# dexmal/dexbotic

Hardware: AMD Instinct MI355X
Metric: episodes/sec DB-CogACT fine-tune (higher is better)
Workload: dtype bf16; 1 GPU; DB-CogACT fine-tune step (CLIP-L/14@224 x1 view, Qwen2.5-7B-class 28L decoder, DiT-B head, AdamW), 16 episodes/GPU, 32-token instruction, S=287; global_batch=16, seq_len=287, parallelism=dp1, optimizer=AdamW serial, grad_accum=1, activations=resident

## Files before the change

### dexbotic_amd/csrc/gemm.hip

```cpp
#include "common.h"
#include "gemm_common.h"

#include <algorithm>

namespace {


template <typename T> struct EltTraits;
template <> struct EltTraits<float> { static constexpr int EPC = 4; };
template <> struct EltTraits<bf16_t> { static constexpr int EPC = 8; };

__device__ __forceinline__ int lds_off(int row, int chunk) { return row * ROWB + ((chunk ^ (row & 7)) << 4); }

template <typename T, int NR>
__device__ __forceinline__ void load_kc(uint4 (&r)[4], const T* __restrict__ base, int64_t ld, int64_t row0,
                                        int64_t rows, int64_t k0, int64_t K, int vec, int tid) {
  constexpr int EPC = EltTraits<T>::EPC;
  const int c = tid & 7;
  const int64_t k = k0 + (int64_t)c * EPC;
#pragma unroll
  for (int i = 0; i < NR / 32; ++i) {
    const int64_t row = row0 + (tid >> 3) + 32 * i;
    uint4 v = make_uint4(0, 0, 0, 0);
    if (row < rows && k < K) {
      const T* p = base + row * ld + k;
      if (vec && k + EPC <= K) {
        v = *reinterpret_cast<const uint4*>(p);
      } else {
        alignas(16) T tmp[EPC];
#pragma unroll
        for (int e = 0; e < EPC; ++e) tmp[e] = (k + e < K) ? p[e] : (T)0;
        v = *reinterpret_cast<const uint4*>(tmp);
      }
    }
    r[i] = v;
  }
}
template <int NR>
__device__ __forceinline__ void store_kc(const uint4 (&r)[4], char* tile, int tid) {
  const int c = tid & 7;
#pragma unroll
  for (int i = 0; i < NR / 32; ++i) {
    const int row = (tid >> 3) + 32 * i;
    *reinterpret_cast<uint4*>(tile + lds_off(row, c)) = r[i];
  }
}

template <typename T> struct KsRegs;
template <> struct KsRegs<bf16_t> { uint2 v[8]; };
template <> struct KsRegs<float> { uint4 v[4]; };

template <typename T, int NR>
__device__ __forceinline__ void load_ks(KsRegs<T>& r, const T* __restrict__ base, int64_t ld, int64_t row0,
                                        int64_t rows, int64_t k0, int64_t K, int vec, int tid) {
  constexpr int EPC = EltTraits<T>::EPC;
  const int kg = tid & 7;
  const int64_t rr = row0 + 4 * (tid >> 3);
#pragma unroll
  for (int j = 0; j < EPC; ++j) {
    const int64_t k = k0 + kg * EPC + j;
    alignas(16) T tmp[4] = {(T)0, (T)0, (T)0, (T)0};
    if (k < K && rr < rows && 4 * (tid >> 3) < NR) {
      const T* p = base + k * ld + rr;
      if (vec && rr + 3 < rows) {
        if constexpr (sizeof(T) == 2) {
          *reinterpret_cast<uint2*>(tmp) = *reinterpret_cast<const uint2*>(p);
        } else {
          *reinterpret_cast<uint4*>(tmp) = *reinterpret_cast<const uint4*>(p);
        }
      } else {
#pragma unroll
        for (int q = 0; q < 4; ++q) tmp[q] = (rr + q < rows) ? p[q] : (T)0;
      }
    }
    if constexpr (sizeof(T) == 2) {
      r.v[j] = *reinterpret_cast<const uint2*>(tmp);
    } else {
      r.v[j] = *reinterpret_cast<const uint4*>(tmp);
    }
  }
}
__device__ __forceinline__ uint32_t half_of(const uint2& v, int q) {
  const uint32_t w = (q & 2) ? v.y : v.x;
  return (q & 1) ? (w >> 16) : (w & 0xffffu);
}
template <int NR>
__device__ __forceinline__ void store_ks(const KsRegs<bf16_t>& r, char* tile, int tid) {
  const int kg = tid & 7;
  if (4 * (tid >> 3) >= NR) return;
#pragma unroll
  for (int q = 0; q < 4; ++q) {
    const int row = 4 * (tid >> 3) + q;
    uint4 o;
    o.x = half_of(r.v[0], q) | (half_of(r.v[1], q) << 16);
    o.y = half_of(r.v[2], q) | (half_of(r.v[3], q) << 16);
    o.z = half_of(r.v[4], q) | (half_of(r.v[5], q) << 16);
    o.w = half_of(r.v[6], q) | (half_of(r.v[7], q) << 16);
    *reinterpret_cast<uint4*>(tile + lds_off(row, kg)) = o;
  }
}
__device__ __forceinline__ uint32_t comp_of(const uint4& v, int q) {
  return q == 0 ? v.x : (q == 1 ? v.y : (q == 2 ? v.z : v.w));
}
template <int NR>
__device__ __forceinline__ void store_ks(const KsRegs<float>& r, char* tile, int tid) {
  const int kg = tid & 7;
  if (4 * (tid >> 3) >= NR) return;
#pragma unroll
  for (int q = 0; q < 4; ++q) {
    const int row = 4 * (tid >> 3) + q;
    uint4 o = make_uint4(comp_of(r.v[0], q), comp_of(r.v[1], q), comp_of(r.v[2], q), comp_of(r.v[3], q));
    *reinterpret_cast<uint4*>(tile + lds_off(row, kg)) = o;
  }
}

template <typename T, bool KS, int NR> struct Stager;
template <typename T, int NR> struct Stager<T, false, NR> {
  uint4 r[4];
  __device__ __forceinline__ void load(const T* base, int64_t ld, int64_t row0, int64_t rows, int64_t k0,
                                       int64_t K, int vec, int tid) {
    load_kc<T, NR>(r, base, ld, row0, rows, k0, K, vec, tid);
  }
  __device__ __forceinline__ void store(char* tile, int tid) { store_kc<NR>(r, tile, tid); }
};
template <typename T, int NR> struct Stager<T, true, NR> {
  KsRegs<T> r;
  __device__ __forceinline__ void load(const T* base, int64_t ld, int64_t row0, int64_t rows, int64_t k0,
                                       int64_t K, int vec, int tid) {
    load_ks<T, NR>(r, base, ld, row0, rows, k0, K, vec, tid);
  }
  __device__ __forceinline__ void store(char* tile, int tid) { store_ks<NR>(r, tile, tid); }
};

template <typename T>
__device__ __forceinline__ void mma_step(f32x4_t& acc, const uint4& first, const uint4& second);
template <>
__device__ __forceinline__ void mma_step<bf16_t>(f32x4_t& acc, const uint4& first, const uint4& second) {
  acc = __builtin_amdgcn_mfma_f32_16x16x32_bf16(__builtin_bit_cast(bf16x8_t, first),
                                                __builtin_bit_cast(bf16x8_t, second), acc, 0, 0, 0);
}
template <>
__device__ __forceinline__ void mma_step<float>(f32x4_t& acc, const uint4& first, const uint4& second) {
  acc = __builtin_amdgcn_mfma_f32_16x16x4f32(__uint_as_float(first.x), __uint_as_float(second.x), acc, 0, 0, 0);
  acc = __builtin_amdgcn_mfma_f32_16x16x4f32(__uint_as_float(first.y), __uint_as_float(second.y), acc, 0, 0, 0);
  acc = __builtin_amdgcn_mfma_f32_16x16x4f32(__uint_as_float(first.z), __uint_as_float(second.z), acc, 0, 0, 0);
  acc = __builtin_amdgcn_mfma_f32_16x16x4f32(__uint_as_float(first.w), __uint_as_float(second.w), acc, 0, 0, 0);
}


template <typename TI, typename TO, bool A_KS, bool B_KS, int TM>
__global__ __launch_bounds__(256) void gemm_kernel(const GemmP p) {
  constexpr int BT = 32 * TM;
  constexpr int TILE_B = BT * ROWB;
  extern __shared__ __attribute__((aligned(16))) char smem[];
  const int tid = threadIdx.x;
  const int lane = tid & 63, wave = tid >> 6;
  const int wm = wave >> 1, wn = wave & 1;
  const int l16 = lane & 15, lg = lane >> 4;

  const int nt = p.tm * p.tn;
  int bid = blockIdx.x;
  {
    const int q = nt >> 3, r = nt & 7, xcd = bid & 7;
    bid = (xcd < r ? xcd * (q + 1) : r * (q + 1) + (xcd - r) * q) + (bid >> 3);
  }
  constexpr int GROUP_M = 8;
  const int width = GROUP_M * p.tn;
  const int group = bid / width;
  const int first_pm = group * GROUP_M;
  const int gsz = min(p.tm - first_pm, GROUP_M);
  const int pm = first_pm + (bid % width) % gsz;
  const int pn = (bid % width) / gsz;
  const int64_t m0 = (int64_t)pm * BT, n0 = (int64_t)pn * BT;

  const int z = blockIdx.z;
  const int b2 = z % p.nb2, b1 = (z / p.nb2) % p.nb1, b0 = z / (p.nb2 * p.nb1);
  const TI* A = reinterpret_cast<const TI*>(p.A) + b0 * p.sA[0] + b1 * p.sA[1] + b2 * p.sA[2];
  const TI* B = reinterpret_cast<const TI*>(p.B) + b0 * p.sB[0] + b1 * p.sB[1] + b2 * p.sB[2];
  const int64_t offC = b0 * p.sC[0] + b1 * p.sC[1] + b2 * p.sC[2];

  constexpr int EPC = EltTraits<TI>::EPC;
  constexpr int BK = 8 * EPC;
  const int64_t nk = (p.K + BK - 1) / BK;

  f32x4_t acc[TM][TM];
#pragma unroll
  for (int i = 0; i < TM; ++i)
#pragma unroll
    for (int j = 0; j < TM; ++j) acc[i][j] = (f32x4_t){0.f, 0.f, 0.f, 0.f};

  Stager<TI, A_KS, BT> sa;
  Stager<TI, B_KS, BT> sb;
  sa.load(A, p.lda, m0, p.M, 0, p.K, p.vecA, tid);
  sb.load(B, p.ldb, n0, p.N, 0, p.K, p.vecB, tid);
  sa.store(smem, tid);
  sb.store(smem + TILE_B, tid);
  __syncthreads();

  for (int64_t kt = 0; kt < nk; ++kt) {
    const int cur = (int)(kt & 1);
    char* As = smem + cur * 2 * TILE_B;
    char* Bs = As + TILE_B;
    const bool more = kt + 1 < nk;
    if (more) {
      sa.load(A, p.lda, m0, p.M, (kt + 1) * BK, p.K, p.vecA, tid);
      sb.load(B, p.ldb, n0, p.N, (kt + 1) * BK, p.K, p.vecB, tid);
    }
#pragma unroll
    for (int s = 0; s < 2; ++s) {
      uint4 af[TM], bfr[TM];
#pragma unroll
      for (int i = 0; i < TM; ++i) {
        af[i] = *reinterpret_cast<const uint4*>(As + lds_off(wm * 16 * TM + i * 16 + l16, 4 * s + lg));
        bfr[i] = *reinterpret_cast<const uint4*>(Bs + lds_off(wn * 16 * TM + i * 16 + l16, 4 * s + lg));
      }
#pragma unroll
      for (int mi = 0; mi < TM; ++mi)
#pragma unroll
        for (int ni = 0; ni < TM; ++ni) mma_step<TI>(acc[mi][ni], bfr[ni], af[mi]);
    }
    if (more) {
      char* An = smem + (cur ^ 1) * 2 * TILE_B;
      sa.store(An, tid);
      sb.store(An + TILE_B, tid);
    }
    __syncthreads();
  }

  TO* C = reinterpret_cast<TO*>(p.C) + offC;
  TO* AUX = p.aux ? reinterpret_cast<TO*>(p.aux) + offC : nullptr;
  const TI* R = p.R ? reinterpret_cast<const TI*>(p.R) + b0 * p.sR[0] + b1 * p.sR[1] + b2 * p.sR[2] : nullptr;
  const TI* G = p.G ? reinterpret_cast<const TI*>(p.G) + b0 * p.sG[0] + b1 * p.sG[1] + b2 * p.sG[2] : nullptr;
  const TI* bias = reinterpret_cast<const TI*>(p.bias);
#pragma unroll
  for (int ni = 0; ni < TM; ++ni) {
    const int64_t n = n0 + wn * 16 * TM + ni * 16 + 4 * lg;
    if (n >= p.N) continue;
    const int n_ok = (int)min((int64_t)4, p.N - n);
    float bv[4] = {0.f, 0.f, 0.f, 0.f};
    if (bias) load4<TI>(bv, bias + n, p.vecBias, n_ok);
#pragma unroll
    for (int mi = 0; mi < TM; ++mi) {
      const int64_t m = m0 + wm * 16 * TM + mi * 16 + l16;
      if (m >= p.M) continue;
      const float a4[4] = {acc[mi][ni][0], acc[mi][ni][1], acc[mi][ni][2], acc[mi][ni][3]};
      epilogue4<TI, TO>(p, C, AUX, R, G, bv, m, n, n_ok, a4);
    }
  }
}

template <typename TO, int NS, int WS, typename TE = bf16_t>
__global__ __launch_bounds__(256 + 64 * WS) void gemm_nt_t128_kernel(const GemmP p) {
#if defined(__HIP_DEVICE_COMPILE__)
  extern __shared__ __attribute__((aligned(16))) char smem[];
  constexpr int STAGE = 32768, A_ST = 16384;
  const int tid = threadIdx.x, lane = tid & 63;
  const int wave_id = __builtin_amdgcn_readfirstlane(tid >> 6);
  const bool loader = WS ? wave_id >= 4 : true;
  const bool worker = WS ? wave_id < 4 : true;
  const int wave = wave_id & 3;
  constexpr int NLW = WS ? WS : 4;
  constexpr int DPW = 16 / NLW;
  const int lw = WS ? (wave_id - 4 < 0 ? 0 : wave_id - 4) : wave_id;
  const int wm = wave >> 1, wn = wave & 1;
  const int l32 = lane & 31, lh = lane >> 5;
  const int nt = p.tm * p.tn;
  const int split_s = p.split_s > 1 ? p.split_s : 1;
  const int split_j = (int)blockIdx.x / nt;
  int bid = (int)blockIdx.x - split_j * nt;
  {
    const int q = nt >> 3, r = nt & 7, xcd = bid & 7;
    bid = (xcd < r ? xcd * (q + 1) : r * (q + 1) + (xcd - r) * q) + (bid >> 3);
  }
  const int pm = bid % p.tm, pn = bid / p.tm;
  const int m0 = pm * 128, n0 = pn * 128;
  const __amdgpu_buffer_rsrc_t rA = __builtin_amdgcn_make_buffer_rsrc(const_cast<char*>(p.A), 0, (int)(((p.M - 1) * p.lda + p.K) * 2), 0x00020000);
  const __amdgpu_buffer_rsrc_t rB = __builtin_amdgcn_make_buffer_rsrc(const_cast<char*>(p.B), 0, (int)(((p.N - 1) * p.ldb + p.K) * 2), 0x00020000);
  uint32_t voA[DPW], voB[DPW];
#pragma unroll
  for (int j = 0; j < DPW; ++j) {
    const int row = (lw * DPW + j) * 8 + (lane >> 3);
    const uint32_t ch = (uint32_t)(((lane & 7) ^ ((row >> 1) & 7)) << 4);
    const int ga = m0 + row, gb = n0 + row;
    voA[j] = ga < (int)p.M ? (uint32_t)ga * (uint32_t)p.lda * 2u + ch : 0x80000000u;
    voB[j] = gb < (int)p.N ? (uint32_t)gb * (uint32_t)p.ldb * 2u + ch : 0x80000000u;
  }
  const int nk_tot = (int)(p.K >> 6);
  const int k_lo = split_j * nk_tot / split_s;
  const int nk = (split_j + 1) * nk_tot / split_s - k_lo;
#define T1_DMA(slot, t)                                                                                                  \
  do {                                                                                                                   \
    _Pragma("unroll") for (int j_ = 0; j_ < DPW; ++j_) {                                                                 \
      __builtin_amdgcn_raw_ptr_buffer_load_lds(rA, (lds_void_t*)(smem + (slot) * STAGE + (lw * DPW + j_) * 1024), 16, voA[j_], (k_lo + (t)) * 128, 0, 0); \
      __builtin_amdgcn_raw_ptr_buffer_load_lds(rB, (lds_void_t*)(smem + (slot) * STAGE + A_ST + (lw * DPW + j_) * 1024), 16, voB[j_], (k_lo + (t)) * 128, 0, 0); \
    }                                                                                                                    \
  } while (0)
  f32x16_t acc[2][2];
#pragma unroll
  for (int i = 0; i < 2; ++i)
#pragma unroll
    for (int j = 0; j < 2; ++j)
#pragma unroll
      for (int r = 0; r < 16; ++r) acc[i][j][r] = 0.f;
  const uint32_t lds0 = (uint32_t)(uintptr_t)(__attribute__((address_space(3))) char*)smem;
  const int sw = (l32 >> 1) & 7;
  const uint32_t ya = (lds0 + (wm * 64 + l32) * 128) | (uint32_t)((lh ^ sw) << 4);
  const uint32_t yb = (lds0 + A_ST + (wn * 64 + l32) * 128) | (uint32_t)((lh ^ sw) << 4);
#define T1_READ(dst, addr, imm) asm volatile("ds_read_b128 %0, %1 offset:%2" : "=v"(dst) : "v"(addr), "n"(imm) : "memory")
#define T1_SB() __builtin_amdgcn_sched_barrier(0)
  if (loader) {
#pragma unroll
    for (int s = 0; s < NS - 1; ++s)
      if (s < nk) T1_DMA(s, s);
  }
  for (int t = 0; t < nk; ++t) {
    const int rem = nk - 1 - t;
    if (loader) {
      if (NS >= 4 && rem >= 2) { if (DPW == 4) asm volatile("s_waitcnt vmcnt(16)" ::: "memory"); else asm volatile("s_waitcnt vmcnt(8)" ::: "memory"); }
      else if (NS >= 3 && rem >= 1) { if (DPW == 4) asm volatile("s_waitcnt vmcnt(8)" ::: "memory"); else asm volatile("s_waitcnt vmcnt(4)" ::: "memory"); }
      else asm volatile("s_waitcnt vmcnt(0)" ::: "memory");
    }
    T1_SB();
    __builtin_amdgcn_s_barrier();
    T1_SB();
    if (loader && t + NS - 1 < nk) T1_DMA((t + NS - 1) % NS, t + NS - 1);
    T1_SB();
    if (!worker) continue;
    const uint32_t so = (uint32_t)((t % NS) * STAGE);
    const uint32_t a_s = ya + so, b_s = yb + so;
    u32x4_t af[2][2], bf[2][2];
    T1_READ(af[0][0], a_s, 0); T1_READ(af[0][1], a_s, 4096); T1_READ(bf[0][0], b_s, 0); T1_READ(bf[0][1], b_s, 4096);
#pragma unroll
    for (int ks = 0; ks < 4; ++ks) {
      const int c = ks & 1, nx = c ^ 1;
      if (ks < 3) {
        const uint32_t a_k = a_s ^ (uint32_t)((ks + 1) << 5), b_k = b_s ^ (uint32_t)((ks + 1) << 5);
        T1_READ(af[nx][0], a_k, 0); T1_READ(af[nx][1], a_k, 4096); T1_READ(bf[nx][0], b_k, 0); T1_READ(bf[nx][1], b_k, 4096);
        asm volatile("s_waitcnt lgkmcnt(4)" ::: "memory");
      } else {
        asm volatile("s_waitcnt lgkmcnt(0)" ::: "memory");
      }
      T1_SB();
#pragma unroll
      for (int i = 0; i < 2; ++i)
#pragma unroll
        for (int j = 0; j < 2; ++j)
          acc[i][j] = __builtin_amdgcn_mfma_f32_32x32x16_bf16(__builtin_bit_cast(bf16x8_t, bf[c][j]), __builtin_bit_cast(bf16x8_t, af[c][i]), acc[i][j], 0, 0, 0);
      T1_SB();
    }
  }
#undef T1_DMA
#undef T1_READ
#undef T1_SB
  if (split_s > 1) {
    constexpr int SC1 = 16;
    constexpr uint32_t SLOT = 128 * 128 * 4;
    const __amdgpu_buffer_rsrc_t rW = __builtin_amdgcn_make_buffer_rsrc(p.ws, 0, (int)(1024u * SLOT), 0x00020000);
    const uint32_t slot0 = (uint32_t)bid * (uint32_t)(split_s - 1) * SLOT + (uint32_t)(tid & 255) * 16u;
    if (split_j < split_s - 1) {
      if (worker)
#pragma unroll
      for (int i = 0; i < 2; ++i)
#pragma unroll
        for (int j = 0; j < 2; ++j)
#pragma unroll
          for (int q = 0; q < 4; ++q) {
            const f32x4_t v = {acc[i][j][4 * q], acc[i][j][4 * q + 1], acc[i][j][4 * q + 2], acc[i][j][4 * q + 3]};
            __builtin_amdgcn_raw_buffer_store_b128(__builtin_bit_cast(u32x4_t, v), rW,
                                                   slot0 + (uint32_t)split_j * SLOT + ((i * 2 + j) * 4 + q) * 4096, 0, SC1);
          }
      asm volatile("s_waitcnt vmcnt(0)" ::: "memory");
      __syncthreads();
      if (tid == 0) __hip_atomic_fetch_add(p.flags + bid, 1, __ATOMIC_RELAXED, __HIP_MEMORY_SCOPE_AGENT);
      return;
    }
    if (tid == 0) {
      while (__hip_atomic_load(p.flags + bid, __ATOMIC_RELAXED, __HIP_MEMORY_SCOPE_AGENT) < split_s - 1)
        __builtin_amdgcn_s_sleep(4);
      __hip_atomic_store(p.flags + bid, 0, __ATOMIC_RELAXED, __HIP_MEMORY_SCOPE_AGENT);
    }
    __syncthreads();
    if (worker)
    for (int sj = 0; sj < split_s - 1; ++sj) {
#pragma unroll
      for (int i = 0; i < 2; ++i)
#pragma unroll
        for (int j = 0; j < 2; ++j)
#pragma unroll
          for (int q = 0; q < 4; ++q) {
            const f32x4_t v = __builtin_bit_cast(f32x4_t, __builtin_amdgcn_raw_buffer_load_b128(
                rW, slot0 + (uint32_t)sj * SLOT + ((i * 2 + j) * 4 + q) * 4096, 0, SC1));
#pragma unroll
            for (int c = 0; c < 4; ++c) acc[i][j][4 * q + c] += v[c];
          }
    }
  }
  if (!worker) return;
  TO* C = reinterpret_cast<TO*>(p.C);
  TO* AUX = p.aux ? reinterpret_cast<TO*>(p.aux) : nullptr;
  const TE* R = reinterpret_cast<const TE*>(p.R);
  const TE* G = reinterpret_cast<const TE*>(p.G);
  const TE* bias = reinterpret_cast<const TE*>(p.bias);
#pragma unroll
  for (int j = 0; j < 2; ++j)
#pragma unroll
    for (int q = 0; q < 4; ++q) {
      const int64_t n = n0 + wn * 64 + 32 * j + 8 * q + 4 * lh;
      if (n >= p.N) continue;
      const int n_ok = (int)min((int64_t)4, p.N - n);
      float bv[4] = {0.f, 0.f, 0.f, 0.f};
      if (bias) load4<TE>(bv, bias + n, p.vecBias, n_ok);
#pragma unroll
      for (int i = 0; i < 2; ++i) {
        const int64_t m = m0 + wm * 64 + 32 * i + l32;
        if (m >= p.M) continue;
        const float a4[4] = {acc[i][j][4 * q], acc[i][j][4 * q + 1], acc[i][j][4 * q + 2], acc[i][j][4 * q + 3]};
        epilogue4<TE, TO>(p, C, AUX, R, G, bv, m, n, n_ok, a4);
      }
    }
#endif
}
template __global__ void gemm_nt_t128_kernel<bf16_t, 4, 4>(const GemmP);
template __global__ void gemm_nt_t128_kernel<float, 4, 4>(const GemmP);

constexpr int GV_MAXM = 8;
template <int M_>
__global__ __launch_bounds__(256) void gemv_nn_stage1_k(const bf16_t* __restrict__ A, int64_t lda, const bf16_t* __restrict__ W,
                                                        int64_t ldb, float* __restrict__ part, int M, int64_t N, int64_t K,
                                                        int kper) {
  __shared__ float as[GV_MAXM][512];
  const int ks = blockIdx.y;
  const int64_t k0 = (int64_t)ks * kper, k1 = min(K, k0 + kper);
  for (int i = threadIdx.x; i < M_ * kper; i += 256) {
    const int m = i / kper, kk = i - m * kper;
    as[m][kk] = (m < M && k0 + kk < k1) ? bf2f(A[(int64_t)m * lda + k0 + kk]) : 0.f;
  }
  __syncthreads();
  const int64_t n = ((int64_t)blockIdx.x * 256 + threadIdx.x) * 8;
  if (n >= N) return;
  float acc[M_][8];
#pragma unroll
  for (int m = 0; m < M_; ++m)
#pragma unroll
    for (int e = 0; e < 8; ++e) acc[m][e] = 0.f;
  const bf16_t* wp = W + k0 * ldb + n;
  const int nkk = (int)(k1 - k0);
  int kk = 0;
  for (; kk + 4 <= nkk; kk += 4) {
    float w[4][8];
#pragma unroll
    for (int u = 0; u < 4; ++u) Vec<bf16_t, 8>::ld(w[u], wp + (int64_t)(kk + u) * ldb);
#pragma unroll
    for (int u = 0; u < 4; ++u)
#pragma unroll
      for (int m = 0; m < M_; ++m) {
        const float a = as[m][kk + u];
#pragma unroll
        for (int e = 0; e < 8; ++e) acc[m][e] += a * w[u][e];
      }
  }
  for (; kk < nkk; ++kk) {
    float w[8];
    Vec<bf16_t, 8>::ld(w, wp + (int64_t)kk * ldb);
#pragma unroll
    for (int m = 0; m < M_; ++m) {
      const float a = as[m][kk];
#pragma unroll
      for (int e = 0; e < 8; ++e) acc[m][e] += a * w[e];
    }
  }
#pragma unroll
  for (int m = 0; m < M_; ++m)
    if (m < M) {
      float* pp = part + ((int64_t)ks * M + m) * N + n;
      *reinterpret_cast<float4*>(pp) = make_float4(acc[m][0], acc[m][1], acc[m][2], acc[m][3]);
      *reinterpret_cast<float4*>(pp + 4) = make_float4(acc[m][4], acc[m][5], acc[m][6], acc[m][7]);
    }
}
template <typename TO>
__global__ __launch_bounds__(256) void gemv_nn_stage2_k(const float* __restrict__ part, TO* __restrict__ C, int64_t ldc, int M,
                                                        int64_t N, int ksplit, float alpha) {
  const int64_t i = (int64_t)blockIdx.x * 256 + threadIdx.x;
  if (i >= (int64_t)M * N) return;
  const int64_t m = i / N, n = i - m * N;
  float s = 0.f;
  for (int ks = 0; ks < ksplit; ++ks) s += part[((int64_t)ks * M + m) * N + n];
  stf<TO>(C + m * ldc + n, s * alpha);
}

template <int MB>
__global__ __launch_bounds__(512) void gemm_skinny_f32_kernel(const GemmP p) {
  __shared__ float red[8][MB][64][4];
  const int tid = threadIdx.x, lane = tid & 63, wave = tid >> 6;
  const int l16 = lane & 15, lg = lane >> 4;
  const int split_s = p.split_s > 1 ? p.split_s : 1;
  const int ntile = (int)gridDim.x / split_s;
  const int tile = (int)blockIdx.x % ntile, split_j = (int)blockIdx.x / ntile;
  const int64_t n0 = (int64_t)tile * 16;
  const float* W = reinterpret_cast<const float*>(p.B) + min(n0 + l16, p.N - 1) * p.ldb + 4 * lg;
  const float* A[MB];
#pragma unroll
  for (int mb = 0; mb < MB; ++mb)
    A[mb] = reinterpret_cast<const float*>(p.A) + min((int64_t)mb * 16 + l16, p.M - 1) * p.lda + 4 * lg;
  f32x4_t acc[MB];
#pragma unroll
  for (int mb = 0; mb < MB; ++mb) acc[mb] = (f32x4_t){0.f, 0.f, 0.f, 0.f};
  const int nkb = (int)(p.K / 64);
  const int kb_lo = split_j * nkb / split_s, kb_hi = (split_j + 1) * nkb / split_s;
  auto ld = [&](int kb, float4 (&wv)[4], float4 (&av)[MB][4]) {
    const int k0 = kb * 64;
#pragma unroll
    for (int j = 0; j < 4; ++j) wv[j] = *reinterpret_cast<const float4*>(W + k0 + 16 * j);
#pragma unroll
    for (int mb = 0; mb < MB; ++mb)
#pragma unroll
      for (int j = 0; j < 4; ++j) av[mb][j] = *reinterpret_cast<const float4*>(A[mb] + k0 + 16 * j);
  };
  auto mma = [&](const float4 (&wv)[4], const float4 (&av)[MB][4]) {
#pragma unroll
    for (int j = 0; j < 4; ++j)
#pragma unroll
      for (int mb = 0; mb < MB; ++mb) {
        acc[mb] = __builtin_amdgcn_mfma_f32_16x16x4f32(wv[j].x, av[mb][j].x, acc[mb], 0, 0, 0);
        acc[mb] = __builtin_amdgcn_mfma_f32_16x16x4f32(wv[j].y, av[mb][j].y, acc[mb], 0, 0, 0);
        acc[mb] = __builtin_amdgcn_mfma_f32_16x16x4f32(wv[j].z, av[mb][j].z, acc[mb], 0, 0, 0);
        acc[mb] = __builtin_amdgcn_mfma_f32_16x16x4f32(wv[j].w, av[mb][j].w, acc[mb], 0, 0, 0);
      }
  };
  for (int kb = kb_lo + wave; kb < kb_hi; kb += 8) {
    float4 w0[4], a0[MB][4];
    ld(kb, w0, a0);
    mma(w0, a0);
  }
#pragma unroll
  for (int mb = 0; mb < MB; ++mb)
    *reinterpret_cast<float4*>(red[wave][mb][lane]) = make_float4(acc[mb][0], acc[mb][1], acc[mb][2], acc[mb][3]);
  __syncthreads();
  const bool worker = wave < MB;
  float a4[4] = {0.f, 0.f, 0.f, 0.f};
  if (worker) {
#pragma unroll
    for (int w = 0; w < 8; ++w) {
      const float4 v = *reinterpret_cast<const float4*>(red[w][wave][lane]);
      a4[0] += v.x; a4[1] += v.y; a4[2] += v.z; a4[3] += v.w;
    }
  }
  if (split_s > 1) {
    constexpr int SC1 = 16;
    constexpr uint32_t SLOT = MB * 64 * 16;
    const __amdgpu_buffer_rsrc_t rW = __builtin_amdgcn_make_buffer_rsrc(p.ws, 0, (int)(256u * 7u * 4u * 64u * 16u), 0x00020000);
    const uint32_t slot0 = (uint32_t)tile * (uint32_t)(split_s - 1) * SLOT + (uint32_t)(wave * 64 + lane) * 16u;
    if (split_j < split_s - 1) {
      if (worker) {
        const f32x4_t v = {a4[0], a4[1], a4[2], a4[3]};
        __builtin_amdgcn_raw_buffer_store_b128(__builtin_bit_cast(u32x4_t, v), rW, slot0 + (uint32_t)split_j * SLOT, 0, SC1);
      }
      asm volatile("s_waitcnt vmcnt(0)" ::: "memory");
      __syncthreads();
      if (tid == 0) __hip_atomic_fetch_add(p.flags + tile, 1, __ATOMIC_RELAXED, __HIP_MEMORY_SCOPE_AGENT);
      return;
    }
    if (tid == 0) {
      while (__hip_atomic_load(p.flags + tile, __ATOMIC_RELAXED, __HIP_MEMORY_SCOPE_AGENT) < split_s - 1)
        __builtin_amdgcn_s_sleep(2);
      __hip_atomic_store(p.flags + tile, 0, __ATOMIC_RELAXED, __HIP_MEMORY_SCOPE_AGENT);
    }
    __syncthreads();
    if (worker) {
      float own[4] = {a4[0], a4[1], a4[2], a4[3]};
      a4[0] = a4[1] = a4[2] = a4[3] = 0.f;
      for (int sj = 0; sj < split_s - 1; ++sj) {
        const f32x4_t v = __builtin_bit_cast(f32x4_t, __builtin_amdgcn_raw_buffer_load_b128(rW, slot0 + (uint32_t)sj * SLOT, 0, SC1));
        a4[0] += v[0]; a4[1] += v[1]; a4[2] += v[2]; a4[3] += v[3];
      }
      a4[0] += own[0]; a4[1] += own[1]; a4[2] += own[2]; a4[3] += own[3];
    }
  }
  if (!worker) return;
  const int64_t m = (int64_t)wave * 16 + l16, n = n0 + 4 * lg;
  if (m >= p.M || n >= p.N) return;
  const int n_ok = (int)min((int64_t)4, p.N - n);
  float bv[4] = {0.f, 0.f, 0.f, 0.f};
  const float* bias = reinterpret_cast<const float*>(p.bias);
  if (bias) load4<float>(bv, bias + n, p.vecBias, n_ok);
  epilogue4<float, float>(p, reinterpret_cast<float*>(p.C), reinterpret_cast<float*>(p.aux),
                          reinterpret_cast<const float*>(p.R), reinterpret_cast<const float*>(p.G), bv, m, n, n_ok, a4);
}

template <int MB, typename TO, int U = 2>
__global__ __launch_bounds__(512) void gemm_skinny_bf16_kernel(const GemmP p) {
  __shared__ float red[8][MB][64][4];
  const int tid = threadIdx.x, lane = tid & 63, wave = tid >> 6;
  const int l16 = lane & 15, lg = lane >> 4;
  const int split_s = p.split_s > 1 ? p.split_s : 1;
  const int ntile = (int)gridDim.x / split_s;
  const int tile = (int)blockIdx.x % ntile, split_j = (int)blockIdx.x / ntile;
  const int64_t n0 = (int64_t)tile * 16;
  const bf16_t* W = reinterpret_cast<const bf16_t*>(p.B) + min(n0 + l16, p.N - 1) * p.ldb + 8 * lg;
  const bf16_t* A[MB];
#pragma unroll
  for (int mb = 0; mb < MB; ++mb)
    A[mb] = reinterpret_cast<const bf16_t*>(p.A) + min((int64_t)mb * 16 + l16, p.M - 1) * p.lda + 8 * lg;
  f32x4_t acc[MB];
#pragma unroll
  for (int mb = 0; mb < MB; ++mb) acc[mb] = (f32x4_t){0.f, 0.f, 0.f, 0.f};
  const int nkb = (int)(p.K / 64);
  const int kb_lo = split_j * nkb / split_s, kb_hi = (split_j + 1) * nkb / split_s;
  for (int kb = kb_lo + wave; kb < kb_hi; kb += 8 * U) {
    u32x4n_t wv[U][2];
    uint4 av[U][MB][2];
#pragma unroll
    for (int u = 0; u < U; ++u) {
      const int k0 = (kb + 8 * u) * 64;
      if (kb + 8 * u < kb_hi) {
#pragma unroll
        for (int j = 0; j < 2; ++j) wv[u][j] = __builtin_nontemporal_load(reinterpret_cast<const u32x4n_t*>(W + k0 + 32 * j));
#pragma unroll
        for (int mb = 0; mb < MB; ++mb)
#pragma unroll
          for (int j = 0; j < 2; ++j) av[u][mb][j] = *reinterpret_cast<const uint4*>(A[mb] + k0 + 32 * j);
      } else {
#pragma unroll
        for (int j = 0; j < 2; ++j) {
          wv[u][j] = (u32x4n_t){0u, 0u, 0u, 0u};
#pragma unroll
          for (int mb = 0; mb < MB; ++mb) av[u][mb][j] = make_uint4(0, 0, 0, 0);
        }
      }
    }
#pragma unroll
    for (int u = 0; u < U; ++u)
#pragma unroll
      for (int j = 0; j < 2; ++j)
#pragma unroll
        for (int mb = 0; mb < MB; ++mb)
          acc[mb] = __builtin_amdgcn_mfma_f32_16x16x32_bf16(__builtin_bit_cast(bf16x8_t, wv[u][j]),
                                                            __builtin_bit_cast(bf16x8_t, av[u][mb][j]), acc[mb], 0, 0, 0);
  }
#pragma unroll
  for (int mb = 0; mb < MB; ++mb)
    *reinterpret_cast<float4*>(red[wave][mb][lane]) = make_float4(acc[mb][0], acc[mb][1], acc[mb][2], acc[mb][3]);
  __syncthreads();
  const bool worker = wave < MB;
  float a4[4] = {0.f, 0.f, 0.f, 0.f};
  if (worker) {
#pragma unroll
    for (int w = 0; w < 8; ++w) {
      const float4 v = *reinterpret_cast<const float4*>(red[w][wave][lane]);
      a4[0] += v.x; a4[1] += v.y; a4[2] += v.z; a4[3] += v.w;
    }
  }
  if (split_s > 1) {
    constexpr int SC1 = 16;
    constexpr uint32_t SLOT = MB * 64 * 16;
    const __amdgpu_buffer_rsrc_t rW = __builtin_amdgcn_make_buffer_rsrc(p.ws, 0, (int)(256u * 7u * 4u * 64u * 16u), 0x00020000);
    const uint32_t slot0 = (uint32_t)tile * (uint32_t)(split_s - 1) * SLOT + (uint32_t)(wave * 64 + lane) * 16u;
    if (split_j < split_s - 1) {
      if (worker) {
        const f32x4_t v = {a4[0], a4[1], a4[2], a4[3]};
        __builtin_amdgcn_raw_buffer_store_b128(__builtin_bit_cast(u32x4_t, v), rW, slot0 + (uint32_t)split_j * SLOT, 0, SC1);
      }
      asm volatile("s_waitcnt vmcnt(0)" ::: "memory");
      __syncthreads();
      if (tid == 0) __hip_atomic_fetch_add(p.flags + tile, 1, __ATOMIC_RELAXED, __HIP_MEMORY_SCOPE_AGENT);
      return;
    }
    if (tid == 0) {
      while (__hip_atomic_load(p.flags + tile, __ATOMIC_RELAXED, __HIP_MEMORY_SCOPE_AGENT) < split_s - 1)
        __builtin_amdgcn_s_sleep(2);
      __hip_atomic_store(p.flags + tile, 0, __ATOMIC_RELAXED, __HIP_MEMORY_SCOPE_AGENT);
    }
    __syncthreads();
    if (worker) {
      const float own[4] = {a4[0], a4[1], a4[2], a4[3]};
      a4[0] = a4[1] = a4[2] = a4[3] = 0.f;
      for (int sj = 0; sj < split_s - 1; ++sj) {
        const f32x4_t v = __builtin_bit_cast(f32x4_t, __builtin_amdgcn_raw_buffer_load_b128(rW, slot0 + (uint32_t)sj * SLOT, 0, SC1));
        a4[0] += v[0]; a4[1] += v[1]; a4[2] += v[2]; a4[3] += v[3];
      }
      a4[0] += own[0]; a4[1] += own[1]; a4[2] += own[2]; a4[3] += own[3];
    }
  }
  if (!worker) return;
  const int64_t m = (int64_t)wave * 16 + l16, n = n0 + 4 * lg;
  if (m >= p.M || n >= p.N) return;
  const int n_ok = (int)min((int64_t)4, p.N - n);
  float bv[4] = {0.f, 0.f, 0.f, 0.f};
  const bf16_t* bias = reinterpret_cast<const bf16_t*>(p.bias);
  if (bias) load4<bf16_t>(bv, bias + n, p.vecBias, n_ok);
  epilogue4<bf16_t, TO>(p, reinterpret_cast<TO*>(p.C), reinterpret_cast<TO*>(p.aux), reinterpret_cast<const bf16_t*>(p.R),
                        reinterpret_cast<const bf16_t*>(p.G), bv, m, n, n_ok, a4);
}


template <typename TO, int AI, typename TE>
__global__ __launch_bounds__(512) void gemm_nt_ring_kernel(const GemmP p) {
#if defined(__HIP_DEVICE_COMPILE__)
  extern __shared__ __attribute__((aligned(16))) char smem[];
  constexpr int A_ST = 256 * 64, STAGE = 2 * A_ST;
  constexpr int BMR = AI * 64;
  const int tid = threadIdx.x, lane = tid & 63;
  const int wave = __builtin_amdgcn_readfirstlane(tid >> 6);
  const int wm = wave >> 2, wn = wave & 3;
  const int l32 = lane & 31, lh = lane >> 5;

  int bid = blockIdx.x;
  int split_j = 0, split_s = 1, tail_i = 0;
  if (bid < p.full) {
    const int q = p.full >> 3, r = p.full & 7, xcd = bid & 7;
    bid = (xcd < r ? xcd * (q + 1) : r * (q + 1) + (xcd - r) * q) + (bid >> 3);
  } else {
    const int idx = bid - p.full;
    tail_i = idx % p.tail_r;
    split_j = idx / p.tail_r;
    split_s = p.split_s;
    bid = p.full + tail_i;
  }
  const int GROUP_M = p.group_m;
  const int width = GROUP_M * p.tn;
  const int group = bid / width;
  const int first_pm = group * GROUP_M;
  const int gsz = min(p.tm - first_pm, GROUP_M);
  const int pm = first_pm + (bid % width) % gsz;
  const int pn = (bid % width) / gsz;
  const int64_t m0 = (int64_t)pm * BMR, n0 = (int64_t)pn * 256;
  const bool has_a = AI == 4 || wave < 6;

  const uint32_t bytesA = (uint32_t)(((p.M - 1) * p.lda + p.K) * 2);
  const uint32_t bytesB = (uint32_t)(((p.N - 1) * p.ldb + p.K) * 2);
  const __amdgpu_buffer_rsrc_t rA = __builtin_amdgcn_make_buffer_rsrc(const_cast<char*>(p.A), 0, bytesA, 0x00020000);
  const __amdgpu_buffer_rsrc_t rB = __builtin_amdgcn_make_buffer_rsrc(const_cast<char*>(p.B), 0, bytesB, 0x00020000);
  uint32_t offA[2], offB[2];
#pragma unroll
  for (int j = 0; j < 2; ++j) {
    const int row = (wave * 2 + j) * 16 + (lane >> 2);
    const int chunk = (lane & 3) ^ ((row >> 2) & 3);
    const int64_t ga = m0 + row, gb = n0 + row;
    offA[j] = ga < p.M ? (uint32_t)((ga * p.lda) * 2 + chunk * 16) : 0x80000000u;
    offB[j] = gb < p.N ? (uint32_t)((gb * p.ldb) * 2 + chunk * 16) : 0x80000000u;
  }
  const int nk_tot = (int)(p.K / 32);
  const int k_lo = (int)((int64_t)split_j * nk_tot / split_s);
  const int nk = (int)((int64_t)(split_j + 1) * nk_tot / split_s) - k_lo;
#define DMA_A(slab, j) __builtin_amdgcn_raw_ptr_buffer_load_lds(rA, (lds_void_t*)(smem + ((slab) & 3) * STAGE + (wave * 2 + (j)) * 1024), 16, offA[j], (k_lo + (slab)) * 64, 0, 0)
#define DMA_B(slab, j) __builtin_amdgcn_raw_ptr_buffer_load_lds(rB, (lds_void_t*)(smem + ((slab) & 3) * STAGE + A_ST + (wave * 2 + (j)) * 1024), 16, offB[j], (k_lo + (slab)) * 64, 0, 0)
#define DMA_SLAB(slab) do { if (has_a) { DMA_A(slab, 0); DMA_A(slab, 1); } DMA_B(slab, 0); DMA_B(slab, 1); } while (0)
#define WAIT_PREV_SLAB() do { if (has_a) asm volatile("s_waitcnt vmcnt(4)" ::: "memory"); else asm volatile("s_waitcnt vmcnt(2)" ::: "memory"); } while (0)

  f32x16_t acc[AI][2];
#pragma unroll
  for (int i = 0; i < AI; ++i)
#pragma unroll
    for (int j = 0; j < 2; ++j)
#pragma unroll
      for (int r = 0; r < 16; ++r) acc[i][j][r] = 0.f;

  DMA_SLAB(0);
  if (nk > 1) DMA_SLAB(1);
  if (nk > 2) {
    DMA_SLAB(2);
    WAIT_PREV_SLAB();
  } else {
    asm volatile("s_waitcnt vmcnt(0)" ::: "memory");
  }
  __builtin_amdgcn_s_barrier();
  __builtin_amdgcn_sched_barrier(0);

  u32x4_t a0[AI], b0[2], a1[AI], b1[2];
  const uint32_t lds0 = (uint32_t)(uintptr_t)(__attribute__((address_space(3))) char*)smem;
  const int sw = (l32 >> 2) & 3;
  const uint32_t abase0 = lds0 + (wm * (BMR / 2) + l32) * 64 + (((0 + lh) ^ sw) << 4);
  const uint32_t abase1 = lds0 + (wm * (BMR / 2) + l32) * 64 + (((2 + lh) ^ sw) << 4);
  const uint32_t bbase0 = lds0 + A_ST + (wn * 64 + l32) * 64 + (((0 + lh) ^ sw) << 4);
  const uint32_t bbase1 = lds0 + A_ST + (wn * 64 + l32) * 64 + (((2 + lh) ^ sw) << 4);
#define DS_READ(dst, addr, imm) asm volatile("ds_read_b128 %0, %1 offset:%2" : "=v"(dst) : "v"(addr), "n"(imm) : "memory")
#define RD_SET(A_, B_, abase, bbase, soff)                                                      \
  do {                                                                                          \
    const uint32_t ax_ = (abase) + (soff), bx_ = (bbase) + (soff);                              \
    DS_READ(A_[0], ax_, 0); DS_READ(A_[1], ax_, 2048); DS_READ(A_[2], ax_, 4096);          \
    if constexpr (AI > 3) DS_READ(A_[3], ax_, 6144);                                            \
    DS_READ(B_[0], bx_, 0); DS_READ(B_[1], bx_, 2048);                                          \
  } while (0)
#define MFMA1(A_, B_, i, j) acc[i][j] = __builtin_amdgcn_mfma_f32_32x32x16_bf16(__builtin_bit_cast(bf16x8_t, B_[j]), __builtin_bit_cast(bf16x8_t, A_[i]), acc[i][j], 0, 0, 0)
#define SB() __builtin_amdgcn_sched_barrier(0)

  RD_SET(a0, b0, abase0, bbase0, 0u);
  for (int t = 0; t < nk; ++t) {
    const uint32_t soff = (uint32_t)((t & 3) * STAGE), soff_n = (uint32_t)(((t + 1) & 3) * STAGE);
    const bool dma = t + 3 < nk;
    asm volatile("s_waitcnt lgkmcnt(0)" ::: "memory");
    SB();
    MFMA1(a0, b0, 0, 0); MFMA1(a0, b0, 0, 1);
    SB();
    RD_SET(a1, b1, abase1, bbase1, soff);
    SB();
    MFMA1(a0, b0, 1, 0); MFMA1(a0, b0, 1, 1);
    SB();
    if (dma && has_a) { DMA_A(t + 3, 0); DMA_A(t + 3, 1); }
    SB();
    MFMA1(a0, b0, 2, 0); MFMA1(a0, b0, 2, 1);
    SB();
    if (dma) { DMA_B(t + 3, 0); DMA_B(t + 3, 1); }
    SB();
    if constexpr (AI > 3) { MFMA1(a0, b0, 3, 0); MFMA1(a0, b0, 3, 1); }
    SB();
    asm volatile("s_waitcnt lgkmcnt(0)" ::: "memory");
    SB();
    MFMA1(a1, b1, 0, 0); MFMA1(a1, b1, 0, 1);
    SB();
    if (t + 1 < nk) RD_SET(a0, b0, abase0, bbase0, soff_n);
    SB();
    MFMA1(a1, b1, 1, 0); MFMA1(a1, b1, 1, 1);
    MFMA1(a1, b1, 2, 0); MFMA1(a1, b1, 2, 1);
    if constexpr (AI > 3) { MFMA1(a1, b1, 3, 0); MFMA1(a1, b1, 3, 1); }
    SB();
    if (dma) WAIT_PREV_SLAB();
    else asm volatile("s_waitcnt vmcnt(0)" ::: "memory");
    __builtin_amdgcn_s_barrier();
    SB();
  }
#undef DMA_A
#undef DMA_B
#undef DMA_SLAB
#undef WAIT_PREV_SLAB
#undef DS_READ
#undef RD_SET
#undef MFMA1
#undef SB

  tile_finish<TO, AI, TE>(p, acc, smem, tid, lane, wave, wm, wn, l32, lh, m0, n0, split_j, split_s, tail_i);
#endif
}
template __global__ void gemm_nt_ring_kernel<bf16_t, 4, bf16_t>(const GemmP);
template __global__ void gemm_nt_ring_kernel<float, 4, bf16_t>(const GemmP);
template __global__ void gemm_nt_ring_kernel<bf16_t, 3, bf16_t>(const GemmP);
template __global__ void gemm_nt_ring_kernel<float, 3, bf16_t>(const GemmP);
template __global__ void gemm_nt_ring_kernel<float, 4, float>(const GemmP);
template __global__ void gemm_nt_ring_kernel<float, 3, float>(const GemmP);


template <typename TO, typename TE, bool LEAN, bool A_KS, bool B_KS, int FUSE = 0>
__global__ __launch_bounds__(512) void gemm_pp_kernel(const GemmP p) {
#if defined(__HIP_DEVICE_COMPILE__)
  extern __shared__ __attribute__((aligned(16))) char smem[];
  constexpr int REG = 256 * 128;
  constexpr int BUF = 2 * REG;
  const int tid = threadIdx.x, lane = tid & 63;
  const int wave = __builtin_amdgcn_readfirstlane(tid >> 6);
  const int wm = wave >> 2, wn = wave & 3;
  const int l32 = lane & 31, lh = lane >> 5;

  int bid = blockIdx.x;
  int split_j = 0, split_s = 1, tail_i = 0;
  if (bid < p.full) {
    const int q = p.full >> 3, r = p.full & 7, xcd = bid & 7;
    bid = (xcd < r ? xcd * (q + 1) : r * (q + 1) + (xcd - r) * q) + (bid >> 3);
  } else {
    const int idx = bid - p.full;
    tail_i = idx % p.tail_r;
    split_j = idx / p.tail_r;
    split_s = p.split_s;
    bid = p.full + tail_i;
  }
  int m0i, n0i;
  sk_tile_origin(p, bid, m0i, n0i);
  const int64_t m0 = m0i, n0 = n0i;

  const uint32_t bytesA = (uint32_t)((A_KS ? (p.K - 1) * p.lda + p.M : (p.M - 1) * p.lda + p.K) * 2);
  const uint32_t bytesB = (uint32_t)((B_KS ? (p.K - 1) * p.ldb + p.N : (p.N - 1) * p.ldb + p.K) * 2);
  const __amdgpu_buffer_rsrc_t rA = __builtin_amdgcn_make_buffer_rsrc(const_cast<char*>(p.A), 0, bytesA, 0x00020000);
  const __amdgpu_buffer_rsrc_t rB = __builtin_amdgcn_make_buffer_rsrc(const_cast<char*>(p.B), 0, bytesB, 0x00020000);
#define PP_A_ROW0(h, j) ((((wave * 2 + (j)) & 7) * 8) + (((wave * 2 + (j)) >> 3) * 128) + 64 * (h))
#define PP_B_ROW0(h, j) ((((wave * 2 + (j)) >> 2) * 64) + (((wave * 2 + (j)) & 3) * 8) + 32 * (h))
  uint32_t voA[2][2], voB[2][2];
  {
    const int lrow = lane >> 3, lslot = lane & 7;
    const uint32_t lda2 = (uint32_t)p.lda * 2u, ldb2 = (uint32_t)p.ldb * 2u;
#pragma unroll
    for (int h = 0; h < 2; ++h)
#pragma unroll
      for (int j = 0; j < 2; ++j) {
        const int krow = (wave * 2 + j) * 4 + (lane >> 4);
        const int sig = (lane & 15) ^ ((krow & 3) << 2);
        if constexpr (A_KS) {
          const int ga = m0i + (sig >> 3) * 128 + 64 * h + 8 * (sig & 7);
          voA[h][j] = ga < (int)p.M ? (uint32_t)krow * lda2 + (uint32_t)ga * 2u : 0x80000000u;
        } else {
          const int ra = PP_A_ROW0(h, j) + lrow, ga = m0i + ra;
          voA[h][j] = ga < (int)p.M ? (uint32_t)ga * lda2 + (uint32_t)((lslot ^ ((ra >> 1) & 7)) << 4) : 0x80000000u;
        }
        if constexpr (B_KS) {
          const int gb = n0i + (sig >> 2) * 64 + 32 * h + 8 * (sig & 3);
          voB[h][j] = gb < (int)p.N ? (uint32_t)krow * ldb2 + (uint32_t)gb * 2u : 0x80000000u;
        } else if constexpr (FUSE == 1) {
          const int rb = PP_B_ROW0(h, j) + lrow, half_n = (int)(p.N >> 1);
          const int lc = (n0i >> 1) + (rb >> 6) * 32 + (rb & 31), gb = ((rb >> 5) & 1) * half_n + lc;
          voB[h][j] = lc < half_n ? (uint32_t)gb * ldb2 + (uint32_t)((lslot ^ ((rb >> 1) & 7)) << 4) : 0x80000000u;
        } else {
          const int rb = PP_B_ROW0(h, j) + lrow, gb = n0i + rb;
          voB[h][j] = gb < (int)p.N ? (uint32_t)gb * ldb2 + (uint32_t)((lslot ^ ((rb >> 1) & 7)) << 4) : 0x80000000u;
        }
      }
  }
  const int nk1 = (int)((p.K + 63) >> 6);
  const int nk_tot = nk1 + ((A_KS && B_KS) ? (int)((p.K2 + 63) >> 6) : 0);
  const bool seg2 = (A_KS && B_KS) && p.K2 > 0;
  const __amdgpu_buffer_rsrc_t rA2 = __builtin_amdgcn_make_buffer_rsrc(
      const_cast<char*>(seg2 ? p.A2 : p.A), 0, seg2 ? (uint32_t)(((p.K2 - 1) * p.lda + p.M) * 2) : 0u, 0x00020000);
  const __amdgpu_buffer_rsrc_t rB2 = __builtin_amdgcn_make_buffer_rsrc(
      const_cast<char*>(seg2 ? p.B2 : p.B), 0, seg2 ? (uint32_t)(((p.K2 - 1) * p.ldb + p.N) * 2) : 0u, 0x00020000);
  const int k_lo = split_j * nk_tot / split_s;
  const int nk = (split_j + 1) * nk_tot / split_s - k_lo;
  const uint32_t ktileA = A_KS ? 64u * (uint32_t)p.lda * 2u : 0u, ktileB = B_KS ? 64u * (uint32_t)p.ldb * 2u : 0u;
#define PP_DMA(rsrc, vo, ldsoff, buf, soff)                                                                             \
  __builtin_amdgcn_raw_ptr_buffer_load_lds(rsrc, (lds_void_t*)(smem + (buf) * BUF + (ldsoff)), 16, vo, soff, 0, 0)
#define PP_DMA_A1(h, j, buf, tile)                                                                          \
  do {                                                                                                      \
    if constexpr (A_KS && B_KS) {                                                                           \
      const int kt_ = k_lo + (tile);                                                                        \
      if (kt_ < nk1) PP_DMA(rA, voA[h][j] + (uint32_t)kt_ * ktileA, (h) * 16384 + (wave * 2 + (j)) * 1024, buf, 0);          \
      else PP_DMA(rA2, voA[h][j] + (uint32_t)(kt_ - nk1) * ktileA, (h) * 16384 + (wave * 2 + (j)) * 1024, buf, 0);           \
    } else if constexpr (A_KS) {                                                                            \
      const uint32_t kb_ = (uint32_t)(k_lo + (tile)) * ktileA;                                              \
      PP_DMA(rA, voA[h][j] + kb_, (h) * 16384 + (wave * 2 + (j)) * 1024, buf, 0);                           \
    } else {                                                                                                \
      PP_DMA(rA, voA[h][j], PP_A_ROW0(h, j) * 128, buf, (k_lo + (tile)) * 128);                             \
    }                                                                                                       \
  } while (0)
#define PP_DMA_B1(h, j, buf, tile)                                                                          \
  do {                                                                                                      \
    if constexpr (A_KS && B_KS) {                                                                           \
      const int kt_ = k_lo + (tile);                                                                        \
      if (kt_ < nk1) PP_DMA(rB, voB[h][j] + (uint32_t)kt_ * ktileB, REG + (h) * 16384 + (wave * 2 + (j)) * 1024, buf, 0);    \
      else PP_DMA(rB2, voB[h][j] + (uint32_t)(kt_ - nk1) * ktileB, REG + (h) * 16384 + (wave * 2 + (j)) * 1024, buf, 0);     \
    } else if constexpr (B_KS) {                                                                            \
      const uint32_t kb_ = (uint32_t)(k_lo + (tile)) * ktileB;                                              \
      PP_DMA(rB, voB[h][j] + kb_, REG + (h) * 16384 + (wave * 2 + (j)) * 1024, buf, 0);                     \
    } else {                                                                                                \
      PP_DMA(rB, voB[h][j], REG + PP_B_ROW0(h, j) * 128, buf, (k_lo + (tile)) * 128);                       \
    }                                                                                                       \
  } while (0)
#define PP_DMA_A(h, buf, tile) do { PP_DMA_A1(h, 0, buf, tile); PP_DMA_A1(h, 1, buf, tile); } while (0)
#define PP_DMA_B(h, buf, tile) do { PP_DMA_B1(h, 0, buf, tile); PP_DMA_B1(h, 1, buf, tile); } while (0)

  f32x16_t acc[4][2];
#pragma unroll
  for (int i = 0; i < 4; ++i)
#pragma unroll
    for (int j = 0; j < 2; ++j)
#pragma unroll
      for (int r = 0; r < 16; ++r) acc[i][j][r] = 0.f;

  const uint32_t lds0 = (uint32_t)(uintptr_t)(__attribute__((address_space(3))) char*)smem;
  const int sw = (l32 >> 1) & 7;
  const int i16 = lane & 15, tq = (i16 >> 2) & 3, tk = 8 * lh + (i16 >> 2);
  const uint32_t ks_lane = (uint32_t)(tk * 256 + ((lane >> 4) & 1) * 32 + (i16 & 3) * 8);
  const uint32_t ya = A_KS ? lds0 + ks_lane + (uint32_t)(((wm * 2) ^ tq) << 6)
                           : (lds0 + (wm * 128 + l32) * 128) | (uint32_t)((lh ^ sw) << 4);
  const uint32_t yb = B_KS ? lds0 + REG + ks_lane + (uint32_t)((wn ^ tq) << 6)
                           : (lds0 + REG + (wn * 64 + l32) * 128) | (uint32_t)((lh ^ sw) << 4);
  u32x4_t af[2][4], bq[2][4];
  typedef uint32_t u32x2_t __attribute__((ext_vector_type(2)));
#define PP_READ(dst, addr, imm) asm volatile("ds_read_b128 %0, %1 offset:%2" : "=v"(dst) : "v"(addr), "n"(imm) : "memory")
#define PP_READ_TR(dst, addr, imm) asm volatile("ds_read_b64_tr_b16 %0, %1 offset:%2" : "=v"(dst) : "v"(addr), "n"(imm) : "memory")
#define PP_FRAG_TR(dst, addr, imm)                                                       \
  do {                                                                                   \
    u32x2_t lo_ = {0u, 0u}, hi_ = {0u, 0u};                                              \
    PP_READ_TR(lo_, addr, imm); PP_READ_TR(hi_, addr, (imm) + 1024);                     \
    dst = (u32x4_t){lo_[0], lo_[1], hi_[0], hi_[1]};                                     \
  } while (0)
#define PP_RD_A(cur, h)                                                                                     \
  do {                                                                                                      \
    if constexpr (A_KS) {                                                                                   \
      const uint32_t a0_ = ya ^ (uint32_t)((cur) * BUF + (h) * 16384), a1_ = a0_ ^ 64u;                     \
      PP_FRAG_TR(af[0][0], a0_, 0); PP_FRAG_TR(af[1][0], a1_, 0);                                           \
      PP_FRAG_TR(af[0][1], a0_, 4096); PP_FRAG_TR(af[1][1], a1_, 4096);                                     \
      PP_FRAG_TR(af[0][2], a0_, 8192); PP_FRAG_TR(af[1][2], a1_, 8192);                                     \
      PP_FRAG_TR(af[0][3], a0_, 12288); PP_FRAG_TR(af[1][3], a1_, 12288);                                   \
    } else {                                                                                                \
      const uint32_t a0_ = ya ^ (uint32_t)((cur) * BUF), a1_ = ya ^ (uint32_t)((cur) * BUF + 32),           \
                     a2_ = ya ^ (uint32_t)((cur) * BUF + 64), a3_ = ya ^ (uint32_t)((cur) * BUF + 96);      \
      PP_READ(af[0][0], a0_, (2 * (h)) * 4096); PP_READ(af[1][0], a0_, (2 * (h) + 1) * 4096);              \
      PP_READ(af[0][1], a1_, (2 * (h)) * 4096); PP_READ(af[1][1], a1_, (2 * (h) + 1) * 4096);              \
      PP_READ(af[0][2], a2_, (2 * (h)) * 4096); PP_READ(af[1][2], a2_, (2 * (h) + 1) * 4096);              \
      PP_READ(af[0][3], a3_, (2 * (h)) * 4096); PP_READ(af[1][3], a3_, (2 * (h) + 1) * 4096);              \
    }                                                                                                       \
  } while (0)
#define PP_RD_B(cur, j)                                                                                     \
  do {                                                                                                      \
    if constexpr (B_KS) {                                                                                   \
      const uint32_t b0_ = yb ^ (uint32_t)((cur) * BUF + (j) * 16384);                                      \
      PP_FRAG_TR(bq[j][0], b0_, 0); PP_FRAG_TR(bq[j][1], b0_, 4096);                                        \
      PP_FRAG_TR(bq[j][2], b0_, 8192); PP_FRAG_TR(bq[j][3], b0_, 12288);                                    \
    } else {                                                                                                \
      const uint32_t b0_ = yb ^ (uint32_t)((cur) * BUF), b1_ = yb ^ (uint32_t)((cur) * BUF + 32),           \
                     b2_ = yb ^ (uint32_t)((cur) * BUF + 64), b3_ = yb ^ (uint32_t)((cur) * BUF + 96);      \
      PP_READ(bq[j][0], b0_, (j) * 4096); PP_READ(bq[j][1], b1_, (j) * 4096);                               \
      PP_READ(bq[j][2], b2_, (j) * 4096); PP_READ(bq[j][3], b3_, (j) * 4096);                               \
    }                                                                                                       \
  } while (0)
#define PP_MFMA(ii, ks, i, j) acc[i][j] = __builtin_amdgcn_mfma_f32_32x32x16_bf16(__builtin_bit_cast(bf16x8_t, bq[j][ks]), __builtin_bit_cast(bf16x8_t, af[ii][ks]), acc[i][j], 0, 0, 0)
#define PP_SB() __builtin_amdgcn_sched_barrier(0)
#define PP_BAR() do { PP_SB(); __builtin_amdgcn_s_barrier(); PP_SB(); } while (0)
#define PP_COMPUTE(h, j)                                                                          \
  do {                                                                                            \
    asm volatile("s_waitcnt lgkmcnt(0)" ::: "memory");                                            \
    PP_SB();                                                                                      \
    PP_MFMA(0, 0, 2 * (h), j); PP_MFMA(1, 0, 2 * (h) + 1, j);                                     \
    PP_MFMA(0, 1, 2 * (h), j); PP_MFMA(1, 1, 2 * (h) + 1, j);                                     \
    PP_MFMA(0, 2, 2 * (h), j); PP_MFMA(1, 2, 2 * (h) + 1, j);                                     \
    PP_MFMA(0, 3, 2 * (h), j); PP_MFMA(1, 3, 2 * (h) + 1, j);                                     \
    PP_SB();                                                                                      \
  } while (0)
#define PP_RDK_A(cur, h, ks)                                                                                \
  do {                                                                                                      \
    if constexpr (A_KS) {                                                                                   \
      const uint32_t a0_ = ya ^ (uint32_t)((cur) * BUF + (h) * 16384), a1_ = a0_ ^ 64u;                     \
      PP_FRAG_TR(af[0][ks], a0_, 4096 * (ks)); PP_FRAG_TR(af[1][ks], a1_, 4096 * (ks));                     \
    } else {                                                                                                \
      const uint32_t a_ = ya ^ (uint32_t)((cur) * BUF + 32 * (ks));                                         \
      PP_READ(af[0][ks], a_, (2 * (h)) * 4096); PP_READ(af[1][ks], a_, (2 * (h) + 1) * 4096);              \
    }                                                                                                       \
  } while (0)
#define PP_RDK_B(cur, j, ks)                                                                                \
  do {                                                                                                      \
    if constexpr (B_KS) {                                                                                   \
      const uint32_t b0_ = yb ^ (uint32_t)((cur) * BUF + (j) * 16384);                                      \
      PP_FRAG_TR(bq[j][ks], b0_, 4096 * (ks));                                                              \
    } else {                                                                                                \
      const uint32_t b_ = yb ^ (uint32_t)((cur) * BUF + 32 * (ks));                                         \
      PP_READ(bq[j][ks], b_, (j) * 4096);                                                                   \
    }                                                                                                       \
  } while (0)
#define PP_COMPUTE_R(h, j, R)                                                                     \
  do {                                                                                            \
    asm volatile("s_waitcnt lgkmcnt(0)" ::: "memory");                                            \
    PP_SB();                                                                                      \
    PP_MFMA(0, 0, 2 * (h), j); PP_MFMA(1, 0, 2 * (h) + 1, j); PP_SB(); R(0); PP_SB();             \
    PP_MFMA(0, 1, 2 * (h), j); PP_MFMA(1, 1, 2 * (h) + 1, j); PP_SB(); R(1); PP_SB();             \
    PP_MFMA(0, 2, 2 * (h), j); PP_MFMA(1, 2, 2 * (h) + 1, j); PP_SB(); R(2); PP_SB();             \
    PP_MFMA(0, 3, 2 * (h), j); PP_MFMA(1, 3, 2 * (h) + 1, j); PP_SB(); R(3); PP_SB();             \
  } while (0)
#define PP_VMCNT(n) asm volatile("s_waitcnt vmcnt(" #n ")" ::: "memory")
#if defined(DXA_PP_STAMPS)
  uint64_t ts_[8];
  uint32_t iv_[8] = {0u, 0u, 0u, 0u, 0u, 0u, 0u, 0u}, ts_last_ = 0u;
#define PP_STAMP(i) asm volatile("s_memtime %0" : "=s"(ts_[i]))
#define PP_STAMPS_FOLD()                                                                                    \
  do {                                                                                                      \
    asm volatile("s_waitcnt lgkmcnt(0)" ::: "memory");                                                      \
    PP_SB();                                                                                                \
    if (ts_last_ != 0u) iv_[7] += (uint32_t)ts_[0] - ts_last_;                                              \
    _Pragma("unroll") for (int i_ = 0; i_ < 7; ++i_) iv_[i_] += (uint32_t)ts_[i_ + 1] - (uint32_t)ts_[i_];  \
    ts_last_ = (uint32_t)ts_[7];                                                                            \
    PP_SB();                                                                                                \
  } while (0)
#else
#define PP_STAMP(i) do { } while (0)
#define PP_STAMPS_FOLD() do { } while (0)
#endif
#define PP_R_B1(ks) PP_RDK_B(cur_, 1, ks)
#define PP_R_A1(ks) PP_RDK_A(cur_, 1, ks)
#define PP_R_NEXT(ks) do { if (more1) { PP_RDK_A(cur_ ^ 1, 0, ks); PP_RDK_B(cur_ ^ 1, 0, ks); } } while (0)
#define PP_TILE(cur, t)                                                                                     \
  do {                                                                                                      \
    constexpr int cur_ = (cur);                                                                             \
    const bool more1 = (t) + 1 < nk, more2 = (t) + 2 < nk;                                                  \
                                                                                               \
    if (more1) { PP_DMA_A(1, cur_ ^ 1, (t) + 1); PP_SB(); PP_VMCNT(8); } else { PP_VMCNT(0); }              \
    PP_BAR(); PP_STAMP(0); PP_COMPUTE_R(0, 0, PP_R_B1); PP_BAR(); PP_STAMP(1);                              \
                                                                                               \
    if (more2) { PP_DMA_A(0, cur_, (t) + 2); PP_SB(); }                                                     \
    PP_BAR(); PP_STAMP(2); PP_COMPUTE_R(0, 1, PP_R_A1); PP_BAR(); PP_STAMP(3);                              \
                                                                                               \
    if (more2) { PP_DMA_B(0, cur_, (t) + 2); PP_SB(); PP_VMCNT(8); } else if (more1) { PP_VMCNT(4); }       \
    PP_BAR(); PP_STAMP(4); PP_COMPUTE(1, 1); PP_BAR(); PP_STAMP(5);                                         \
                                                                                               \
    if (more2) { PP_DMA_B(1, cur_, (t) + 2); PP_SB(); PP_VMCNT(8); } else if (more1) { PP_VMCNT(2); }       \
    PP_BAR(); PP_STAMP(6); PP_COMPUTE_R(1, 0, PP_R_NEXT); PP_BAR(); PP_STAMP(7);                            \
    PP_STAMPS_FOLD();                                                                                       \
  } while (0)

  PP_DMA_A(0, 0, 0); PP_DMA_B(0, 0, 0); PP_DMA_B(1, 0, 0); PP_DMA_A(1, 0, 0);
  if (nk > 1) { PP_DMA_A(0, 1, 1); PP_DMA_B(0, 1, 1); PP_DMA_B(1, 1, 1); }
  PP_SB();
  if (nk > 1) { PP_VMCNT(8); } else { PP_VMCNT(2); }
  PP_BAR();
  PP_RD_A(0, 0); PP_RD_B(0, 0);
  PP_SB();
  if (wm == 1) PP_BAR();
  for (int t = 0; t < nk; t += 2) {
    PP_TILE(0, t);
    if (t + 1 < nk) PP_TILE(1, t + 1);
  }
  if (wm == 0) PP_BAR();
#if defined(DXA_PP_STAMPS)
  const uint32_t iv0_ = iv_[0], iv1_ = iv_[1], iv2_ = iv_[2], iv3_ = iv_[3], iv4_ = iv_[4], iv5_ = iv_[5], iv6_ = iv_[6], iv7_ = iv_[7];
#endif
#undef PP_A_ROW0
#undef PP_B_ROW0
#undef PP_DMA
#undef PP_DMA_A
#undef PP_DMA_B
#undef PP_READ
#undef PP_READ_TR
#undef PP_FRAG_TR
#undef PP_RD_A
#undef PP_RD_B
#undef PP_MFMA
#undef PP_SB
#undef PP_BAR
#undef PP_COMPUTE
#undef PP_VMCNT
#undef PP_TILE
#undef PP_DMA_A1
#undef PP_DMA_B1
#undef PP_STAMP
#undef PP_STAMPS_FOLD
#undef PP_RDK_A
#undef PP_RDK_B
#undef PP_COMPUTE_R
#undef PP_R_B1
#undef PP_R_A1
#undef PP_R_NEXT

  if constexpr (LEAN) {
    if (!tile_split_exchange<4>(p, acc, tid, split_j, split_s, tail_i)) return;
    __builtin_amdgcn_sched_barrier(0);
    if constexpr (FUSE == 1) sk_epilogue_swiglu<4>(p, acc, smem + wave * 4096, lane, wm, wn, m0i, n0i);
    else sk_epilogue<TO, TE>(p, acc, smem + wave * 4096, lane, wm, wn, m0i, n0i, reinterpret_cast<float*>(smem + 8 * 4096), bid);
#if defined(DXA_PP_STAMPS)
    __syncthreads();
    if (m0i == 0 && n0i == 0 && lane == 0) {
      uint32_t* o_ = reinterpret_cast<uint32_t*>(p.C) + wave * 16;
      o_[0] = iv0_; o_[1] = iv1_; o_[2] = iv2_; o_[3] = iv3_; o_[4] = iv4_; o_[5] = iv5_; o_[6] = iv6_; o_[7] = iv7_;
      o_[8] = (uint32_t)nk;
    }
#endif
  } else {
    tile_finish<TO, 4, TE>(p, acc, smem, tid, lane, wave, wm, wn, l32, lh, m0, n0, split_j, split_s, tail_i);
  }
#endif
}
template __global__ void gemm_pp_kernel<bf16_t, bf16_t, true, false, false>(const GemmP);
template __global__ void gemm_pp_kernel<float, bf16_t, true, false, false>(const GemmP);
template __global__ void gemm_pp_kernel<float, float, true, false, false>(const GemmP);
template __global__ void gemm_pp_kernel<bf16_t, bf16_t, false, false, false>(const GemmP);
template __global__ void gemm_pp_kernel<float, bf16_t, false, false, false>(const GemmP);
template __global__ void gemm_pp_kernel<float, float, false, false, false>(const GemmP);
template __global__ void gemm_pp_kernel<bf16_t, bf16_t, true, false, true>(const GemmP);
template __global__ void gemm_pp_kernel<bf16_t, bf16_t, false, false, true>(const GemmP);
template __global__ void gemm_pp_kernel<float, bf16_t, true, false, true>(const GemmP);
template __global__ void gemm_pp_kernel<float, bf16_t, true, true, true>(const GemmP);
template __global__ void gemm_pp_kernel<bf16_t, bf16_t, true, true, true>(const GemmP);
template __global__ void gemm_pp_kernel<bf16_t, bf16_t, true, false, false, 1>(const GemmP);

#if defined(DXA_PP3_STAMPS)
__device__ unsigned long long g_pp3_stamps[4];
#define P3_STAMP(i) do { if (blockIdx.x == DXA_PP3_STAMPS && threadIdx.x == 0) { unsigned long long t_; asm volatile("s_memtime %0\n\ts_waitcnt lgkmcnt(0)" : "=s"(t_) :: "memory"); g_pp3_stamps[i] = t_; } } while (0)
#else
#define P3_STAMP(i) do { } while (0)
#endif
template <typename TO, typename TE, bool LEAN, int FUSE = 0>
__global__ __launch_bounds__(512) void gemm_pp3_kernel(const GemmP p) {
#if defined(__HIP_DEVICE_COMPILE__)
  extern __shared__ __attribute__((aligned(16))) char smem[];
  P3_STAMP(0);
  constexpr int AREG = 192 * 128, BREG = 256 * 128, BUFSZ = AREG + BREG;
  const int tid = threadIdx.x, lane = tid & 63;
  const int wave = __builtin_amdgcn_readfirstlane(tid >> 6);
  const int wm = wave >> 2, wn = wave & 3;
  const int l32 = lane & 31, lh = lane >> 5;
  int bid = blockIdx.x;
  int split_j = 0, split_s = 1, tail_i = 0;
  if (bid < p.full) {
    const int q = p.full >> 3, r = p.full & 7, xcd = bid & 7;
    bid = (xcd < r ? xcd * (q + 1) : r * (q + 1) + (xcd - r) * q) + (bid >> 3);
  } else {
    const int idx = bid - p.full;
    tail_i = idx % p.tail_r;
    split_j = idx / p.tail_r;
    split_s = p.split_s;
    bid = p.full + tail_i;
  }
  const int width = p.group_m * p.tn;
  const int group = bid / width;
  const int first_pm = group * p.group_m;
  const int gsz = min(p.tm - first_pm, p.group_m);
  const int pm = first_pm + (bid % width) % gsz;
  const int pn = (bid % width) / gsz;
  const int64_t m0 = (int64_t)pm * 192, n0 = (int64_t)pn * 256;

  const uint32_t bytesA = (uint32_t)(((p.M - 1) * p.lda + p.K) * 2);
  const uint32_t bytesB = (uint32_t)(((p.N - 1) * p.ldb + p.K) * 2);
  const __amdgpu_buffer_rsrc_t rA = __builtin_amdgcn_make_buffer_rsrc(const_cast<char*>(p.A), 0, bytesA, 0x00020000);
  const __amdgpu_buffer_rsrc_t rB = __builtin_amdgcn_make_buffer_rsrc(const_cast<char*>(p.B), 0, bytesB, 0x00020000);
#define P3_A_ROW0(g) ((wave >> 2) * 96 + 32 * (g) + (wave & 3) * 8)
#define P3_B_ROW0(h, j) ((((wave * 2 + (j)) >> 2) * 64) + (((wave * 2 + (j)) & 3) * 8) + 32 * (h))
  uint32_t voA[3], voB[2][2];
  {
    const int lrow = lane >> 3, lslot = lane & 7;
    const uint32_t lda2 = (uint32_t)p.lda * 2u, ldb2 = (uint32_t)p.ldb * 2u;
#pragma unroll
    for (int g = 0; g < 3; ++g) {
      const int ra = P3_A_ROW0(g) + lrow;
      const int64_t ga = m0 + ra;
      voA[g] = ga < p.M ? (uint32_t)ga * lda2 + (uint32_t)((lslot ^ ((ra >> 1) & 7)) << 4) : 0x80000000u;
    }
#pragma unroll
    for (int h = 0; h < 2; ++h)
#pragma unroll
      for (int j = 0; j < 2; ++j) {
        const int rb = P3_B_ROW0(h, j) + lrow;
        if constexpr (FUSE == 1) {
          const int half_n = (int)(p.N >> 1);
          const int lc = (int)(n0 >> 1) + (rb >> 6) * 32 + (rb & 31), gb = ((rb >> 5) & 1) * half_n + lc;
          voB[h][j] = lc < half_n ? (uint32_t)gb * ldb2 + (uint32_t)((lslot ^ ((rb >> 1) & 7)) << 4) : 0x80000000u;
        } else {
          const int64_t gb = n0 + rb;
          voB[h][j] = gb < p.N ? (uint32_t)gb * ldb2 + (uint32_t)((lslot ^ ((rb >> 1) & 7)) << 4) : 0x80000000u;
        }
      }
  }
  const int nk_tot = (int)(p.K / 64);
  const int k_lo = split_j * nk_tot / split_s;
  const int nk = (split_j + 1) * nk_tot / split_s - k_lo;
#define P3_DMA(rsrc, vo, ldsoff, buf, tile) \
  __builtin_amdgcn_raw_ptr_buffer_load_lds(rsrc, (lds_void_t*)(smem + (buf) * BUFSZ + (ldsoff)), 16, vo, (k_lo + (tile)) * 128, 0, 0)
#define P3_DMA_A(g, buf, tile) P3_DMA(rA, voA[g], P3_A_ROW0(g) * 128, buf, tile)
#define P3_DMA_B(h, buf, tile) do { P3_DMA(rB, voB[h][0], AREG + P3_B_ROW0(h, 0) * 128, buf, tile); P3_DMA(rB, voB[h][1], AREG + P3_B_ROW0(h, 1) * 128, buf, tile); } while (0)

  f32x16_t acc[3][2];
#pragma unroll
  for (int i = 0; i < 3; ++i)
#pragma unroll
    for (int j = 0; j < 2; ++j)
#pragma unroll
      for (int r = 0; r < 16; ++r) acc[i][j][r] = 0.f;

  const uint32_t lds0 = (uint32_t)(uintptr_t)(__attribute__((address_space(3))) char*)smem;
  const int sw = (l32 >> 1) & 7;
  const uint32_t ya0 = (lds0 + (wm * 96 + l32) * 128) | (uint32_t)((lh ^ sw) << 4), ya1 = ya0 + BUFSZ;
  const uint32_t yb0 = (lds0 + AREG + (wn * 64 + l32) * 128) | (uint32_t)((lh ^ sw) << 4), yb1 = yb0 + BUFSZ;
  u32x4_t af[2][4], bq[2][2][4];
#define P3_READ(dst, addr, imm) asm volatile("ds_read_b128 %0, %1 offset:%2" : "=v"(dst) : "v"(addr), "n"(imm) : "memory")
#define P3_RD_A(buf, g, set, ks) P3_READ(af[set][ks], ((buf) ? ya1 : ya0) ^ (uint32_t)(32 * (ks)), (g) * 4096)
#define P3_RD_B(buf, h, bset, ks) P3_READ(bq[bset][h][ks], ((buf) ? yb1 : yb0) ^ (uint32_t)(32 * (ks)), (h) * 4096)
#define P3_MFMA(g, set, bset, j, ks) acc[g][j] = __builtin_amdgcn_mfma_f32_32x32x16_bf16(__builtin_bit_cast(bf16x8_t, bq[bset][j][ks]), __builtin_bit_cast(bf16x8_t, af[set][ks]), acc[g][j], 0, 0, 0)
#define P3_SB() __builtin_amdgcn_sched_barrier(0)
#define P3_BAR() do { P3_SB(); __builtin_amdgcn_s_barrier(); P3_SB(); } while (0)
#define P3_COMPUTE(g, set, bset, R)                                                                 \
  do {                                                                                              \
    asm volatile("s_waitcnt lgkmcnt(0)" ::: "memory");                                              \
    P3_SB();                                                                                        \
    P3_MFMA(g, set, bset, 0, 0); P3_MFMA(g, set, bset, 1, 0); P3_SB(); R(0); P3_SB();               \
    P3_MFMA(g, set, bset, 0, 1); P3_MFMA(g, set, bset, 1, 1); P3_SB(); R(1); P3_SB();               \
    P3_MFMA(g, set, bset, 0, 2); P3_MFMA(g, set, bset, 1, 2); P3_SB(); R(2); P3_SB();               \
    P3_MFMA(g, set, bset, 0, 3); P3_MFMA(g, set, bset, 1, 3); P3_SB(); R(3); P3_SB();               \
  } while (0)
#define P3_VMCNT(n) asm volatile("s_waitcnt vmcnt(" #n ")" ::: "memory")
#define P3_TILE(cur, t)                                                                                                  \
  do {                                                                                                                   \
    constexpr int cur_ = (cur), s0_ = (cur), s1_ = (cur) ^ 1;            \
    const bool more1 = (t) + 1 < nk, more2 = (t) + 2 < nk;                                                               \
                                                                                                            \
    if (more1) P3_DMA_A(2, cur_ ^ 1, (t) + 1);                                                                           \
    if (more2) { P3_DMA_B(0, cur_, (t) + 2); P3_SB(); P3_VMCNT(7); } else if (more1) { P3_SB(); P3_VMCNT(5); } else { P3_VMCNT(0); } \
    P3_BAR();                                                                                                            \
    P3_COMPUTE(0, s0_, cur_, P3_R_A1);                                                                                   \
    P3_BAR();                                                                                                            \
                                                                                                            \
    if (more2) { P3_DMA_A(0, cur_, (t) + 2); P3_DMA_B(1, cur_, (t) + 2); P3_SB(); P3_VMCNT(7); } else if (more1) { P3_VMCNT(2); } \
    P3_BAR();                                                                                                            \
    P3_COMPUTE(1, s1_, cur_, P3_R_A2B0);                                                                                 \
    P3_BAR();                                                                                                            \
                                                                                                            \
    if (more2) { P3_DMA_A(1, cur_, (t) + 2); P3_SB(); P3_VMCNT(7); } else if (more1) { P3_VMCNT(1); }                    \
    P3_BAR();                                                                                                            \
    P3_COMPUTE(2, s0_, cur_, P3_R_A0B1);                                                                                 \
    P3_BAR();                                                                                                            \
  } while (0)
#define P3_R_A1(ks) P3_RD_A(cur_, 1, s1_, ks)
#define P3_R_A2B0(ks) do { P3_RD_A(cur_, 2, s0_, ks); if (more1) P3_RD_B(cur_ ^ 1, 0, cur_ ^ 1, ks); } while (0)
#define P3_R_A0B1(ks) do { if (more1) { P3_RD_A(cur_ ^ 1, 0, s1_, ks); P3_RD_B(cur_ ^ 1, 1, cur_ ^ 1, ks); } } while (0)

  P3_DMA_B(0, 0, 0); P3_DMA_A(0, 0, 0); P3_DMA_B(1, 0, 0); P3_DMA_A(1, 0, 0); P3_DMA_A(2, 0, 0);
  if (nk > 1) { P3_DMA_B(0, 1, 1); P3_DMA_A(0, 1, 1); P3_DMA_B(1, 1, 1); P3_DMA_A(1, 1, 1); }
  P3_SB();
  if (nk > 1) { P3_VMCNT(7); } else { P3_VMCNT(1); }
  P3_BAR();
  P3_STAMP(1);
#pragma unroll
  for (int ks = 0; ks < 4; ++ks) { P3_RD_A(0, 0, 0, ks); P3_RD_B(0, 0, 0, ks); P3_RD_B(0, 1, 0, ks); }
  P3_SB();
  if (wm == 1) P3_BAR();
  for (int t = 0; t < nk; t += 2) {
    P3_TILE(0, t);
    if (t + 1 < nk) P3_TILE(1, t + 1);
  }
  if (wm == 0) P3_BAR();
  P3_STAMP(2);
#undef P3_A_ROW0
#undef P3_B_ROW0
#undef P3_DMA
#undef P3_DMA_A
#undef P3_DMA_B
#undef P3_READ
#undef P3_RD_A
#undef P3_RD_B
#undef P3_MFMA
#undef P3_SB
#undef P3_BAR
#undef P3_COMPUTE
#undef P3_VMCNT
#undef P3_TILE
#undef P3_R_A1
#undef P3_R_A2B0
#undef P3_R_A0B1
  if constexpr (LEAN) {
    if (!tile_split_exchange<3>(p, acc, tid, split_j, split_s, tail_i)) return;
    __builtin_amdgcn_sched_barrier(0);
    if constexpr (FUSE == 1) sk_epilogue_swiglu<3>(p, acc, smem + wave * 4096, lane, wm, wn, (int)m0, (int)n0);
    else sk_epilogue<TO, TE, 3>(p, acc, smem + wave * 4096, lane, wm, wn, (int)m0, (int)n0, reinterpret_cast<float*>(smem + 8 * 4096), bid);
  } else {
    tile_finish<TO, 3, TE>(p, acc, smem, tid, lane, wave, wm, wn, l32, lh, m0, n0, split_j, split_s, tail_i);
  }
  asm volatile("s_waitcnt vmcnt(0)" ::: "memory");
  P3_STAMP(3);
#endif
}
#undef P3_STAMP
template __global__ void gemm_pp3_kernel<bf16_t, bf16_t, true>(const GemmP);
template __global__ void gemm_pp3_kernel<float, bf16_t, true>(const GemmP);
template __global__ void gemm_pp3_kernel<bf16_t, bf16_t, false>(const GemmP);
template __global__ void gemm_pp3_kernel<float, bf16_t, false>(const GemmP);
template __global__ void gemm_pp3_kernel<float, float, true>(const GemmP);
template __global__ void gemm_pp3_kernel<float, float, false>(const GemmP);
template __global__ void gemm_pp3_kernel<bf16_t, bf16_t, true, 1>(const GemmP);

__global__ __launch_bounds__(256) void split3_k(const float* __restrict__ src, int64_t ld, bf16_t* __restrict__ dst,
                                                int64_t rows, int64_t cols, int side) {
  const int64_t c4 = cols >> 2;
  for (int64_t i = (int64_t)blockIdx.x * 256 + threadIdx.x; i < rows * c4; i += (int64_t)gridDim.x * 256) {
    const int64_t r = i / c4, c = (i - r * c4) * 4;
    float x[4];
    Vec<float, 4>::ld(x, src + r * ld + c);
    float hi[4], lo[4];
#pragma unroll
    for (int e = 0; e < 4; ++e) {
      hi[e] = bf2f(f2bf(x[e]));
      lo[e] = x[e] - hi[e];
    }
    bf16_t* d = dst + r * 3 * cols + c;
    Vec<bf16_t, 4>::st(d, hi);
    Vec<bf16_t, 4>::st(d + cols, side == 0 ? hi : lo);
    Vec<bf16_t, 4>::st(d + 2 * cols, side == 0 ? lo : hi);
  }
}

template <typename TI, typename TO, int TM>
int launch(const GemmP& p, int layout, dim3 grid, hipStream_t st) {
  constexpr size_t LDS = 4 * (32 * TM) * ROWB;
  switch (layout) {
    case DXA_NT: hipLaunchKernelGGL((gemm_kernel<TI, TO, false, false, TM>), grid, dim3(256), LDS, st, p); break;
    case DXA_NN: hipLaunchKernelGGL((gemm_kernel<TI, TO, false, true, TM>), grid, dim3(256), LDS, st, p); break;
    case DXA_TN: hipLaunchKernelGGL((gemm_kernel<TI, TO, true, true, TM>), grid, dim3(256), LDS, st, p); break;
    default: return DXA_ERR_BAD_ARG;
  }
  return DXA_OK;
}

constexpr int NUM_CU = 256;
static_assert(NUM_CU == NUM_CU_D, "split-K scratch sizing");
constexpr size_t SPLIT_WS_BYTES = (size_t)NUM_CU * 256 * 256 * 4;
struct SplitWs { float* ws; int* flags; };
int get_split_ws(hipStream_t st, SplitWs* out) {
  static StreamBlock blocks(SPLIT_WS_BYTES + NUM_CU * sizeof(int));
  char* base = nullptr;
  if (int rc = blocks.get(st, &base)) return rc;
  DXA_CHECK_ARG(base != nullptr, "dxa_gemm: first split-K product on a stream allocates its scratch and cannot happen under stream "
                "capture: run the request once eagerly on this stream first");
  *out = SplitWs{(float*)base, (int*)(base + SPLIT_WS_BYTES)};
  return DXA_OK;
}

constexpr int RING_LDS = 139264;
template <auto kernel>
int launch_ring(dim3 grid, hipStream_t st, const GemmP& p) {
  return dxa_launch_lds<kernel>(RING_LDS, grid, dim3(512), RING_LDS, st, p);
}

inline bool aligned_to(const void* p, size_t a) { return (reinterpret_cast<uintptr_t>(p) % a) == 0; }
inline bool strides_mult(const int64_t s[3], int64_t m) { return s[0] % m == 0 && s[1] % m == 0 && s[2] % m == 0; }

}

namespace {
int gemm_dispatch(const dxa_gemm_desc* d, dxa_stream_t stream, bool* mirrored, bool* summed);

template <typename T>
__global__ __launch_bounds__(256) void sumsq_rows_k(const T* __restrict__ C, int64_t ldc, int64_t M, int64_t N,
                                                    float* __restrict__ out) {
  __shared__ float red[4];
  float s = 0.f;
  for (int64_t r = blockIdx.x; r < M; r += gridDim.x) {
    const T* row = C + r * ldc;
    for (int64_t c = threadIdx.x; c < N; c += 256) { const float v = ldf<T>(row + c); s += v * v; }
  }
#pragma unroll
  for (int o = 32; o > 0; o >>= 1) s += __shfl_xor(s, o, 64);
  if ((threadIdx.x & 63) == 0) red[threadIdx.x >> 6] = s;
  __syncthreads();
  if (threadIdx.x == 0) out[blockIdx.x] = (red[0] + red[1]) + (red[2] + red[3]);
}
}
extern "C" int64_t dxa_gemm_sumsq_slots(int64_t M, int64_t N) {
  if (M <= 0 || N <= 0) return 0;
  return ((M + 255) / 256) * ((N + 255) / 256);
}
extern "C" int dxa_gemm(const dxa_gemm_desc* d, dxa_stream_t stream) {
  bool mirrored = false, summed = false;
  if (int rc = gemm_dispatch(d, stream, &mirrored, &summed)) return rc;
  if (d->mirror && !mirrored && d->M > 0 && d->N > 0) {
    if (int rc = dxa_copy2d(d->C, d->ldc, d->mirror, d->ldc, d->M, d->N, d->N, DXA_F32, DXA_BF16, stream)) return rc;
  }
  if (d->sumsq && !summed && d->M > 0 && d->N > 0) {
    const dim3 sgrid((unsigned)dxa_gemm_sumsq_slots(d->M, d->N));
    if (d->out_dtype == DXA_F32)
      hipLaunchKernelGGL(sumsq_rows_k<float>, sgrid, dim3(256), 0, (hipStream_t)stream, (const float*)d->C, d->ldc, d->M, d->N, d->sumsq);
    else
      hipLaunchKernelGGL(sumsq_rows_k<bf16_t>, sgrid, dim3(256), 0, (hipStream_t)stream, (const bf16_t*)d->C, d->ldc, d->M, d->N, d->sumsq);
    DXA_CHECK_LAUNCH();
  }
  return DXA_OK;
}
namespace {
int gemm_dispatch(const dxa_gemm_desc* d, dxa_stream_t stream, bool* mirrored, bool* summed) {
  DXA_CHECK_ARG(d != nullptr, "dxa_gemm: null desc");
  DXA_CHECK_ARG(d->M >= 0 && d->N >= 0 && d->K >= 0, "dxa_gemm: negative dims");
  DXA_CHECK_ARG(d->layout >= DXA_NT && d->layout <= DXA_TN, "dxa_gemm: bad layout %d", d->layout);
  DXA_CHECK_ARG(d->in_dtype == DXA_F32 || d->in_dtype == DXA_BF16, "dxa_gemm: bad in_dtype %d", d->in_dtype);
  DXA_CHECK_ARG(d->out_dtype == d->in_dtype || d->out_dtype == DXA_F32,
                "dxa_gemm: out_dtype must equal in_dtype or be fp32");
  DXA_CHECK_ARG(d->nb[0] >= 1 && d->nb[1] >= 1 && d->nb[2] >= 1, "dxa_gemm: batch extents must be >= 1");
  if (d->M == 0 || d->N == 0) return DXA_OK;
  DXA_CHECK_ARG(d->A && d->B && d->C, "dxa_gemm: null operand");
  const int64_t nbatch = (int64_t)d->nb[0] * d->nb[1] * d->nb[2];
  DXA_CHECK_ARG(nbatch <= 65535, "dxa_gemm: too many batches (%lld)", (long long)nbatch);

  const size_t es = d->in_dtype == DXA_BF16 ? 2 : 4, os = d->out_dtype == DXA_BF16 ? 2 : 4;
  const int64_t epc = 16 / es;
  if (d->in_dtype == DXA_BF16 && nbatch == 1 && d->layout != DXA_TN && d->K % 64 != 0 && d->K >= 1024 &&
      d->M >= 256 && d->N >= 256 && d->act == DXA_ACT_NONE && !d->aux_out && !d->mulgrad && !d->sumsq && !d->mirror && !d->epi_f32) {
    const int64_t K0 = d->K - d->K % 64;
    dxa_gemm_desc head = *d, tail = *d;
    head.K = K0;
    tail.K = d->K - K0;
    tail.accumulate = 1; tail.bias = nullptr; tail.residual = nullptr;
    tail.A = (const char*)d->A + K0 * (int64_t)es;
    tail.B = (const char*)d->B + (d->layout == DXA_NT ? K0 : K0 * d->ldb) * (int64_t)es;
    bool m2 = false, s2 = false;
    if (int rc = gemm_dispatch(&head, stream, &m2, &s2)) return rc;
    return gemm_dispatch(&tail, stream, &m2, &s2);
  }
  GemmP p;
  memset(&p, 0, sizeof(p));
  p.M = d->M; p.N = d->N; p.K = d->K;
  p.A = (const char*)d->A; p.lda = d->lda;
  p.B = (const char*)d->B; p.ldb = d->ldb;
  p.C = (char*)d->C; p.ldc = d->ldc;
  p.bias = (const char*)d->bias;
  p.R = (const char*)d->residual; p.ldr = d->ldr;
  p.aux = (char*)d->aux_out;
  p.G = (const char*)d->mulgrad; p.ldg = d->ldg;
  p.alpha = d->alpha; p.act = d->act; p.accumulate = d->accumulate;
  p.fuse = d->fuse; p.ldaux = d->ld_aux;
  if (d->fuse != DXA_FUSE_NONE) {
    DXA_CHECK_ARG(d->fuse == DXA_FUSE_SWIGLU, "dxa_gemm: unknown fuse mode %d", d->fuse);
    const int64_t F_ = d->N / 2;
    DXA_CHECK_ARG(d->layout == DXA_NT && d->in_dtype == DXA_BF16 && d->out_dtype == DXA_BF16 && nbatch == 1 && d->N % 2 == 0 &&
                  F_ % 8 == 0 && d->K % 64 == 0 && d->K >= 64 && d->M >= 129 && F_ >= 128 && !d->bias && !d->residual && !d->mulgrad &&
                  d->act == DXA_ACT_NONE && !d->accumulate && !d->mirror && !d->sumsq && !d->epi_f32 && d->K2 == 0,
                  "dxa_gemm: DXA_FUSE_SWIGLU is a plain bf16 NT product of the MFMA fast path (M >= 129, K %% 64 == 0, F %% 8 == 0)");
    DXA_CHECK_ARG(aligned_to(d->A, 16) && aligned_to(d->B, 16) && aligned_to(d->C, 8) && d->lda % 8 == 0 && d->ldb % 8 == 0 &&
                  d->ldc % 4 == 0 && d->ldc >= F_ && (!d->aux_out || (aligned_to(d->aux_out, 8) && d->ld_aux % 4 == 0 && d->ld_aux >= d->N)) &&
                  ((d->M - 1) * d->ld_aux + d->N) * 2 < (1ll << 31) && ((d->M - 1) * d->lda + d->K) * 2 < (1ll << 31) &&
                  ((d->N - 1) * d->ldb + d->K) * 2 < (1ll << 31),
                  "dxa_gemm: DXA_FUSE_SWIGLU needs 16-byte aligned operand rows, 8-byte aligned output rows and operands < 2 GiB");
  }
  DXA_CHECK_ARG(!d->mirror || (d->out_dtype == DXA_F32 && nbatch == 1), "dxa_gemm: mirror needs an fp32, unbatched output");
  DXA_CHECK_ARG(!d->sumsq || nbatch == 1, "dxa_gemm: sumsq needs an unbatched output");
  p.nb1 = d->nb[1]; p.nb2 = d->nb[2];
  for (int i = 0; i < 3; ++i) {
    p.sA[i] = d->sA[i]; p.sB[i] = d->sB[i]; p.sC[i] = d->sC[i]; p.sR[i] = d->sR[i]; p.sG[i] = d->sG[i];
  }
  p.tm = dxa_cdiv(d->M, BM);
  p.tn = dxa_cdiv(d->N, BN);
  const bool a_ks = d->layout == DXA_TN, b_ks = d->layout != DXA_NT;
  p.vecA = a_ks ? (aligned_to(d->A, 4 * es) && d->lda % 4 == 0 && strides_mult(d->sA, 4))
                : (aligned_to(d->A, 16) && d->lda % epc == 0 && strides_mult(d->sA, epc));
  p.vecB = b_ks ? (aligned_to(d->B, 4 * es) && d->ldb % 4 == 0 && strides_mult(d->sB, 4))
                : (aligned_to(d->B, 16) && d->ldb % epc == 0 && strides_mult(d->sB, epc));
  p.vecC = aligned_to(d->C, 4 * os) && d->ldc % 4 == 0 && strides_mult(d->sC, 4) &&
           (!d->aux_out || aligned_to(d->aux_out, 4 * os));
  const size_t ees = d->epi_f32 ? 4 : es;
  DXA_CHECK_ARG(!d->epi_f32 || (d->in_dtype == DXA_BF16 && d->out_dtype == DXA_F32), "dxa_gemm: epi_f32 needs bf16 in, fp32 out");
  p.vecR = d->residual && aligned_to(d->residual, 4 * ees) && d->ldr % 4 == 0 && strides_mult(d->sR, 4);
  p.vecG = d->mulgrad && aligned_to(d->mulgrad, 4 * ees) && d->ldg % 4 == 0 && strides_mult(d->sG, 4);
  p.vecBias = d->bias && aligned_to(d->bias, 4 * ees);

  hipStream_t st = (hipStream_t)stream;
  const int64_t bytesA = (a_ks ? (d->K - 1) * d->lda + d->M : (d->M - 1) * d->lda + d->K) * 2;
  const int64_t bytesB = (b_ks ? (d->K - 1) * d->ldb + d->N : (d->N - 1) * d->ldb + d->K) * 2;
  const bool ks_layout = d->layout != DXA_NT;
  const int64_t cpl = 16 / (int64_t)os;
  const bool lean_ok = d->N % cpl == 0 && d->ldc % cpl == 0 && aligned_to(d->C, 16) &&
                       ((d->M - 1) * d->ldc + d->N) * (int64_t)os < (1ll << 31) && !d->aux_out && !d->mulgrad &&
                       d->act == DXA_ACT_NONE && (!d->bias || aligned_to(d->bias, cpl * ees)) &&
                       (!d->residual || (aligned_to(d->residual, cpl * ees) && d->ldr % cpl == 0 &&
                                         ((d->M - 1) * d->ldr + d->N) * (int64_t)ees < (1ll << 31)));
  const bool ks_ok = (d->layout == DXA_NN ? (d->out_dtype == DXA_BF16 || lean_ok) : lean_ok) && !d->epi_f32 && ks_layout && aligned_to(d->A, 16) && aligned_to(d->B, 16) && d->lda % 8 == 0 && d->ldb % 8 == 0 &&
                     (d->layout == DXA_TN || d->K % 64 == 0) && d->K >= 64;
  const int64_t t128_tiles = (int64_t)dxa_cdiv(d->M, 128) * dxa_cdiv(d->N, 128);
  if (d->fuse == DXA_FUSE_NONE && d->layout == DXA_NT && d->in_dtype == DXA_BF16 && nbatch == 1 && !d->epi_f32 &&
      d->M >= 64 && d->M <= 1024 && d->N >= 64 && d->K >= 64 && d->K % 64 == 0 && p.vecA && p.vecB &&
      bytesA < (1ll << 31) && bytesB < (1ll << 31) && t128_tiles >= 32 && t128_tiles <= NUM_CU && d->K <= 4096) {
    p.tm = dxa_cdiv(d->M, 128);
    p.tn = dxa_cdiv(d->N, 128);
    int t_split = 1;
    if (t128_tiles <= NUM_CU / 4 || (t128_tiles <= NUM_CU / 2 && d->K >= 2048))
      t_split = (int)std::min<int64_t>(std::min<int64_t>(4, NUM_CU / t128_tiles), (d->K / 64) / 8);
    if (t_split >= 2) {
      SplitWs w;
      if (int rc = get_split_ws(st, &w)) return rc;
      p.split_s = t_split; p.ws = w.ws; p.flags = w.flags;
    } else {
      p.split_s = 1;
    }
    dim3 tgrid((unsigned)(p.tm * p.tn * p.split_s));
    constexpr int T128_LDS = 4 * 32768;
    const int rc = d->out_dtype == DXA_BF16
                       ? dxa_launch_lds<gemm_nt_t128_kernel<bf16_t, 4, 4>>(T128_LDS, tgrid, dim3(512), T128_LDS, st, p)
                       : dxa_launch_lds<gemm_nt_t128_kernel<float, 4, 4>>(T128_LDS, tgrid, dim3(512), T128_LDS, st, p);
    if (rc) return rc;
    DXA_CHECK_LAUNCH();
    return DXA_OK;
  }
  if (d->K2 > 0) {
    DXA_CHECK_ARG(d->layout == DXA_TN && d->A2 && d->B2 && nbatch == 1, "dxa_gemm: A2 / B2 / K2 need an unbatched TN product");
    const int64_t bytesA2 = ((d->K2 - 1) * d->lda + d->M) * 2, bytesB2 = ((d->K2 - 1) * d->ldb + d->N) * 2;
    const bool seg_fast = d->in_dtype == DXA_BF16 && ks_ok && d->M >= 64 && d->N >= 64 &&
                          (int64_t)d->M * d->N >= 128 * 128 && bytesA < (1ll << 31) && bytesB < (1ll << 31) &&
                          bytesA2 < (1ll << 31) && bytesB2 < (1ll << 31) && aligned_to(d->A2, 16) && aligned_to(d->B2, 16);
    if (!seg_fast) {
      dxa_gemm_desc first = *d, second = *d;
      first.A2 = first.B2 = nullptr; first.K2 = 0; first.mirror = nullptr; first.sumsq = nullptr;
      second.A = d->A2; second.B = d->B2; second.K = d->K2; second.A2 = second.B2 = nullptr; second.K2 = 0;
      second.accumulate = 1; second.bias = nullptr; second.residual = nullptr;
      bool m1 = false, s1 = false;
      if (int rc = gemm_dispatch(&first, stream, &m1, &s1)) return rc;
      return gemm_dispatch(&second, stream, mirrored, summed);
    }
    p.A2 = (const char*)d->A2; p.B2 = (const char*)d->B2; p.K2 = d->K2;
  }
  if (d->in_dtype == DXA_BF16 && nbatch == 1 &&
      ((d->layout == DXA_NT && d->K >= 32 && d->K % 32 == 0 && p.vecA && p.vecB) || ks_ok) &&
      d->M >= 64 && d->N >= 64 && (int64_t)d->M * d->N >= 128 * 128 && bytesA < (1ll << 31) && bytesB < (1ll << 31)) {
    const int64_t pad256 = (int64_t)dxa_cdiv(d->M, 256) * 256, pad192 = (int64_t)dxa_cdiv(d->M, 192) * 192;
    const int ai = ks_layout ? 4 : (pad192 * 27 < pad256 * 25 ? 3 : 4);
    p.tm = dxa_cdiv(d->M, ai * 64);
    p.tn = dxa_cdiv(d->N, 256);
    const int nt = p.tm * p.tn, nk_tot = (int)((d->K + d->K2 + 31) / 32);
    p.full = nt; p.tail_r = 0; p.split_s = 1;
    p.group_m = 4;
    const int tail = nt % NUM_CU;
    if (tail > 0) {
      const int s = nk_tot >= 64 ? std::min(std::min(NUM_CU / tail, 8), nk_tot / 32) : 1;
      if (s >= 2) {
        SplitWs w;
        if (int rc = get_split_ws(st, &w)) return rc;
        p.full = nt - tail; p.tail_r = tail; p.split_s = s; p.ws = w.ws; p.flags = w.flags;
      }
    }
    dim3 fgrid((unsigned)(p.full + p.tail_r * p.split_s));
    const bool pp = ks_layout || (ai == 4 && d->K % 64 == 0);
    const bool lean = pp && lean_ok;
    const bool bf = d->out_dtype == DXA_BF16;
    if (lean) { p.mirror = (char*)d->mirror; *mirrored = d->mirror != nullptr; }
    if (lean) { p.sumsq = d->sumsq; *summed = d->sumsq != nullptr; }
    int rc;
    if (d->layout == DXA_NN) {
      if (bf) rc = lean ? launch_ring<gemm_pp_kernel<bf16_t, bf16_t, true, false, true>>(fgrid, st, p)
                        : launch_ring<gemm_pp_kernel<bf16_t, bf16_t, false, false, true>>(fgrid, st, p);
      else rc = launch_ring<gemm_pp_kernel<float, bf16_t, true, false, true>>(fgrid, st, p);
    } else if (d->layout == DXA_TN) {
      rc = bf ? launch_ring<gemm_pp_kernel<bf16_t, bf16_t, true, true, true>>(fgrid, st, p)
              : launch_ring<gemm_pp_kernel<float, bf16_t, true, true, true>>(fgrid, st, p);
    } else if (d->fuse == DXA_FUSE_SWIGLU && ai == 4) {
      rc = launch_ring<gemm_pp_kernel<bf16_t, bf16_t, true, false, false, 1>>(fgrid, st, p);
    } else if (d->fuse == DXA_FUSE_SWIGLU) {
      rc = launch_ring<gemm_pp3_kernel<bf16_t, bf16_t, true, 1>>(fgrid, st, p);
    } else if (pp && lean) {
      if (d->epi_f32) rc = launch_ring<gemm_pp_kernel<float, float, true, false, false>>(fgrid, st, p);
      else if (bf) rc = launch_ring<gemm_pp_kernel<bf16_t, bf16_t, true, false, false>>(fgrid, st, p);
      else rc = launch_ring<gemm_pp_kernel<float, bf16_t, true, false, false>>(fgrid, st, p);
    } else if (pp) {
      if (d->epi_f32) rc = launch_ring<gemm_pp_kernel<float, float, false, false, false>>(fgrid, st, p);
      else if (bf) rc = launch_ring<gemm_pp_kernel<bf16_t, bf16_t, false, false, false>>(fgrid, st, p);
      else rc = launch_ring<gemm_pp_kernel<float, bf16_t, false, false, false>>(fgrid, st, p);
    }
    else if (ai == 3 && d->K % 64 == 0 && d->layout == DXA_NT) {
      if (d->epi_f32) rc = lean_ok ? launch_ring<gemm_pp3_kernel<float, float, true>>(fgrid, st, p)
                                   : launch_ring<gemm_pp3_kernel<float, float, false>>(fgrid, st, p);
      else if (lean_ok) rc = bf ? launch_ring<gemm_pp3_kernel<bf16_t, bf16_t, true>>(fgrid, st, p)
                                : launch_ring<gemm_pp3_kernel<float, bf16_t, true>>(fgrid, st, p);
      else rc = bf ? launch_ring<gemm_pp3_kernel<bf16_t, bf16_t, false>>(fgrid, st, p)
                   : launch_ring<gemm_pp3_kernel<float, bf16_t, false>>(fgrid, st, p);
    }
    else if (d->epi_f32) rc = ai == 3 ? launch_ring<gemm_nt_ring_kernel<float, 3, float>>(fgrid, st, p)
                                      : launch_ring<gemm_nt_ring_kernel<float, 4, float>>(fgrid, st, p);
    else if (ai == 3) rc = bf ? launch_ring<gemm_nt_ring_kernel<bf16_t, 3, bf16_t>>(fgrid, st, p)
                              : launch_ring<gemm_nt_ring_kernel<float, 3, bf16_t>>(fgrid, st, p);
    else rc = bf ? launch_ring<gemm_nt_ring_kernel<bf16_t, 4, bf16_t>>(fgrid, st, p)
                 : launch_ring<gemm_nt_ring_kernel<float, 4, bf16_t>>(fgrid, st, p);
    if (rc) return rc;
    DXA_CHECK_LAUNCH();
    return DXA_OK;
  }
  DXA_CHECK_ARG(d->fuse == DXA_FUSE_NONE, "dxa_gemm: fuse is only implemented on the bf16 NT MFMA fast path (K %% 32 == 0, M, N >= 64, 16-byte aligned rows, no batching)");
  DXA_CHECK_ARG(!d->epi_f32, "dxa_gemm: epi_f32 is only implemented on the bf16 NT fast path (K %% 32 == 0, M, N >= 64, "
                              "16-byte aligned rows, no batching)");
  if (d->layout == DXA_NN && d->in_dtype == DXA_BF16 && nbatch == 1 && d->M <= GV_MAXM && d->K >= 64 &&
      d->N >= 64 && d->N % 8 == 0 && d->ldb % 8 == 0 && aligned_to(d->B, 16) && !d->bias && !d->residual && !d->aux_out &&
      !d->mulgrad && d->act == DXA_ACT_NONE && !d->accumulate && !d->epi_f32) {
    const int nbn = dxa_cdiv(d->N, 2048);
    int ksplit = (int)std::min<int64_t>(std::min<int64_t>(64, d->K / 32), dxa_cdiv(512, nbn));
    if (ksplit < 1) ksplit = 1;
    int kper = dxa_cdiv(d->K, ksplit);
    if (kper > 512) { kper = 512; ksplit = dxa_cdiv(d->K, kper); }
    if ((size_t)ksplit * d->M * d->N * sizeof(float) <= (size_t)NUM_CU * 256 * 256 * 4) {
      SplitWs w;
      if (int rc = get_split_ws(st, &w)) return rc;
      dim3 g1((unsigned)nbn, (unsigned)ksplit);
      const bf16_t* A_ = (const bf16_t*)d->A;
      const bf16_t* W_ = (const bf16_t*)d->B;
#define LAUNCH_GV(M_) hipLaunchKernelGGL((gemv_nn_stage1_k<M_>), g1, dim3(256), 0, st, A_, d->lda, W_, d->ldb, w.ws, (int)d->M, d->N, d->K, kper)
      if (d->M <= 1) LAUNCH_GV(1); else if (d->M <= 2) LAUNCH_GV(2); else if (d->M <= 4) LAUNCH_GV(4); else LAUNCH_GV(8);
#undef LAUNCH_GV
      dim3 g2((unsigned)dxa_cdiv(d->M * d->N, 256));
      if (d->out_dtype == DXA_BF16)
        hipLaunchKernelGGL(gemv_nn_stage2_k<bf16_t>, g2, dim3(256), 0, st, w.ws, (bf16_t*)d->C, d->ldc, (int)d->M, d->N, ksplit, d->alpha);
      else
        hipLaunchKernelGGL(gemv_nn_stage2_k<float>, g2, dim3(256), 0, st, w.ws, (float*)d->C, d->ldc, (int)d->M, d->N, ksplit, d->alpha);
      DXA_CHECK_LAUNCH();
      return DXA_OK;
    }
  }
  if (d->layout == DXA_NT && d->in_dtype == DXA_BF16 && nbatch == 1 && d->M <= 64 && d->K >= 64 &&
      d->K % 64 == 0 && p.vecA && p.vecB) {
    const int64_t skb_tiles = dxa_cdiv(d->N, 16);
    int skb_split = 1;
    if (skb_tiles <= NUM_CU / 2)
      skb_split = (int)std::max<int64_t>(1, std::min<int64_t>(std::min<int64_t>(8, (d->K / 64) / 8), dxa_cdiv(256, skb_tiles)));
    p.split_s = 1;
    if (skb_split >= 2) {
      SplitWs w;
      if (int rc = get_split_ws(st, &w)) return rc;
      p.split_s = skb_split; p.ws = w.ws; p.flags = w.flags;
    }
    dim3 sgrid((unsigned)(skb_tiles * p.split_s));
    const int mb = dxa_cdiv(d->M, 16);
#define LAUNCH_SK(MB_, U_)                                                                                          \
  do {                                                                                                              \
    if (d->out_dtype == DXA_BF16) hipLaunchKernelGGL((gemm_skinny_bf16_kernel<MB_, bf16_t, U_>), sgrid, dim3(512), 0, st, p); \
    else hipLaunchKernelGGL((gemm_skinny_bf16_kernel<MB_, float, U_>), sgrid, dim3(512), 0, st, p);               \
  } while (0)
    if (mb == 1) LAUNCH_SK(1, 4); else if (mb == 2) LAUNCH_SK(2, 2); else if (mb == 3) LAUNCH_SK(3, 2); else LAUNCH_SK(4, 2);
#undef LAUNCH_SK
    DXA_CHECK_LAUNCH();
    return DXA_OK;
  }
  if (d->layout == DXA_NT && d->in_dtype == DXA_F32 && d->out_dtype == DXA_F32 && nbatch == 1 &&
      d->M <= 64 && d->K >= 64 && d->K % 64 == 0 && p.vecA && p.vecB) {
    const int64_t sk_tiles = dxa_cdiv(d->N, 16);
    int sk_split = 1;
    if (sk_tiles <= NUM_CU / 2)
      sk_split = (int)std::max<int64_t>(1, std::min<int64_t>(std::min<int64_t>(8, (d->K / 64) / 8), dxa_cdiv(256, sk_tiles)));
    p.split_s = 1;
    if (sk_split >= 2) {
      SplitWs w;
      if (int rc = get_split_ws(st, &w)) return rc;
      p.split_s = sk_split; p.ws = w.ws; p.flags = w.flags;
    }
    dim3 sgrid((unsigned)(sk_tiles * p.split_s));
    switch (dxa_cdiv(d->M, 16)) {
      case 1: hipLaunchKernelGGL((gemm_skinny_f32_kernel<1>), sgrid, dim3(512), 0, st, p); break;
      case 2: hipLaunchKernelGGL((gemm_skinny_f32_kernel<2>), sgrid, dim3(512), 0, st, p); break;
      case 3: hipLaunchKernelGGL((gemm_skinny_f32_kernel<3>), sgrid, dim3(512), 0, st, p); break;
      default: hipLaunchKernelGGL((gemm_skinny_f32_kernel<4>), sgrid, dim3(512), 0, st, p); break;
    }
    DXA_CHECK_LAUNCH();
    return DXA_OK;
  }
  const bool small = (int64_t)p.tm * p.tn * nbatch < 192;
  if (small) {
    p.tm = dxa_cdiv(d->M, 64);
    p.tn = dxa_cdiv(d->N, 64);
  }
  dim3 grid((unsigned)(p.tm * p.tn), 1, (unsigned)nbatch);
  int rc;
  if (d->in_dtype == DXA_BF16) {
    if (small) rc = d->out_dtype == DXA_BF16 ? launch<bf16_t, bf16_t, 2>(p, d->layout, grid, st) : launch<bf16_t, float, 2>(p, d->layout, grid, st);
    else rc = d->out_dtype == DXA_BF16 ? launch<bf16_t, bf16_t, 4>(p, d->layout, grid, st) : launch<bf16_t, float, 4>(p, d->layout, grid, st);
  } else {
    rc = small ? launch<float, float, 2>(p, d->layout, grid, st) : launch<float, float, 4>(p, d->layout, grid, st);
  }
  if (rc != DXA_OK) return rc;
  DXA_CHECK_LAUNCH();
  return DXA_OK;
}
}

namespace {
__global__ __launch_bounds__(256) void split3_t_k(const float* __restrict__ src, int64_t ld, bf16_t* __restrict__ dst, int64_t R,
                                                  int64_t C, int64_t Rp, int side) {
  __shared__ float tile[32][33];
  const int tx = threadIdx.x & 31, ty = threadIdx.x >> 5;
  const int64_t r0 = (int64_t)blockIdx.y * 32, c0 = (int64_t)blockIdx.x * 32;
#pragma unroll
  for (int i = 0; i < 4; ++i) {
    const int64_t r = r0 + ty + 8 * i, c = c0 + tx;
    tile[ty + 8 * i][tx] = (r < R && c < C) ? src[r * ld + c] : 0.f;
  }
  __syncthreads();
#pragma unroll
  for (int i = 0; i < 4; ++i) {
    const int64_t c = c0 + ty + 8 * i, r = r0 + tx;
    if (c < C && r < Rp) {
      const float x = tile[tx][ty + 8 * i];
      const bf16_t hb = f2bf(x);
      const bf16_t lb = f2bf(x - bf2f(hb));
      bf16_t* d = dst + c * 3 * Rp + r;
      d[0] = hb;
      d[Rp] = side == 0 ? hb : lb;
      d[2 * Rp] = side == 0 ? lb : hb;
    }
  }
}
}
extern "C" int dxa_split3_t(const float* src, int64_t ld, void* dst, int64_t R, int64_t C, int64_t Rp, int side,
                            dxa_stream_t stream) {
  DXA_CHECK_ARG(R >= 0 && C >= 0 && Rp >= R && ld >= C && (side == 0 || side == 1), "dxa_split3_t: bad arguments");
  if (Rp == 0 || C == 0) return DXA_OK;
  DXA_CHECK_ARG(src && dst, "dxa_split3_t: null buffer");
  const dim3 grid((unsigned)((C + 31) / 32), (unsigned)((Rp + 31) / 32));
  DXA_CHECK_ARG(grid.y <= 65535, "dxa_split3_t: too many rows");
  hipLaunchKernelGGL(split3_t_k, grid, dim3(256), 0, (hipStream_t)stream, src, ld, (bf16_t*)dst, R, C, Rp, side);
  DXA_CHECK_LAUNCH();
  return DXA_OK;
}
namespace {
struct S3Op { const float* src; int64_t ld; bf16_t* dst; int64_t rows, cols, pad; int side, transposed; unsigned nblocks, tiles_x; };
__global__ __launch_bounds__(256) void split3_pair_k(const S3Op a, const S3Op b) {
  __shared__ float tile[32][33];
  const bool first = blockIdx.x < a.nblocks;
  const S3Op& o = first ? a : b;
  const unsigned bid = first ? blockIdx.x : blockIdx.x - a.nblocks;
  if (!o.transposed) {
    const int64_t c4 = o.cols >> 2;
    for (int64_t i = (int64_t)bid * 256 + threadIdx.x; i < o.rows * c4; i += (int64_t)o.nblocks * 256) {
      const int64_t r = i / c4, c = (i - r * c4) * 4;
      float x[4];
      Vec<float, 4>::ld(x, o.src + r * o.ld + c);
      float hi[4], lo[4];
#pragma unroll
      for (int e = 0; e < 4; ++e) {
        hi[e] = bf2f(f2bf(x[e]));
        lo[e] = x[e] - hi[e];
      }
      bf16_t* d = o.dst + r * 3 * o.cols + c;
      Vec<bf16_t, 4>::st(d, hi);
      Vec<bf16_t, 4>::st(d + o.cols, o.side == 0 ? hi : lo);
      Vec<bf16_t, 4>::st(d + 2 * o.cols, o.side == 0 ? lo : hi);
    }
    return;
  }
  const int tx = threadIdx.x & 31, ty = threadIdx.x >> 5;
  const int64_t R = o.rows, C_ = o.cols, Rp = o.pad;
  const int64_t r0 = (int64_t)(bid / o.tiles_x) * 32, c0 = (int64_t)(bid % o.tiles_x) * 32;
#pragma unroll
  for (int i = 0; i < 4; ++i) {
    const int64_t r = r0 + ty + 8 * i, c = c0 + tx;
    tile[ty + 8 * i][tx] = (r < R && c < C_) ? o.src[r * o.ld + c] : 0.f;
  }
  __syncthreads();
#pragma unroll
  for (int i = 0; i < 4; ++i) {
    const int64_t c = c0 + ty + 8 * i, r = r0 + tx;
    if (c < C_ && r < Rp) {
      const float x = tile[tx][ty + 8 * i];
      const bf16_t hb = f2bf(x);
      const bf16_t lb = f2bf(x - bf2f(hb));
      bf16_t* d = o.dst + c * 3 * Rp + r;
      d[0] = hb;
      d[Rp] = o.side == 0 ? hb : lb;
      d[2 * Rp] = o.side == 0 ? lb : hb;
    }
  }
}
int s3_fill(const dxa_split3_op* u, S3Op* o) {
  DXA_CHECK_ARG(u && u->rows >= 0 && u->cols >= 0 && (u->side == 0 || u->side == 1) && u->ld >= u->cols, "dxa_split3_pair: bad operand");
  o->src = u->src; o->ld = u->ld; o->dst = (bf16_t*)u->dst; o->rows = u->rows; o->cols = u->cols; o->pad = u->pad; o->side = u->side;
  o->transposed = u->transposed != 0; o->nblocks = 0; o->tiles_x = 1;
  if (u->rows == 0 || u->cols == 0) return DXA_OK;
  DXA_CHECK_ARG(u->src && u->dst, "dxa_split3_pair: null buffer");
  if (o->transposed) {
    DXA_CHECK_ARG(u->pad >= u->rows, "dxa_split3_pair: pad < rows");
    o->tiles_x = (unsigned)((u->cols + 31) / 32);
    const int64_t nb = (int64_t)o->tiles_x * ((u->pad + 31) / 32);
    DXA_CHECK_ARG(nb < (1ll << 30), "dxa_split3_pair: operand too large");
    o->nblocks = (unsigned)nb;
  } else {
    DXA_CHECK_ARG(u->cols % 4 == 0 && u->ld % 4 == 0 && (reinterpret_cast<uintptr_t>(u->src) % 16) == 0 &&
                      (reinterpret_cast<uintptr_t>(u->dst) % 8) == 0,
                  "dxa_split3_pair: cols and ld must be multiples of 4 and the buffers 16-byte aligned");
    o->nblocks = (unsigned)dxa_grid1d(u->rows * (u->cols / 4), 256);
  }
  return DXA_OK;
}
}
extern "C" int dxa_split3_pair(const dxa_split3_op* a, const dxa_split3_op* b, dxa_stream_t stream) {
  S3Op oa, ob;
  if (int rc = s3_fill(a, &oa)) return rc;
  if (int rc = s3_fill(b, &ob)) return rc;
  if (oa.nblocks + ob.nblocks == 0) return DXA_OK;
  hipLaunchKernelGGL(split3_pair_k, dim3(oa.nblocks + ob.nblocks), dim3(256), 0, (hipStream_t)stream, oa, ob);
  DXA_CHECK_LAUNCH();
  return DXA_OK;
}
extern "C" int dxa_split3(const float* src, int64_t ld, void* dst, int64_t rows, int64_t cols, int side, dxa_stream_t stream) {
  DXA_CHECK_ARG(rows >= 0 && cols >= 0 && (side == 0 || side == 1), "dxa_split3: bad arguments");
  if (rows == 0 || cols == 0) return DXA_OK;
  DXA_CHECK_ARG(src && dst, "dxa_split3: null buffer");
  DXA_CHECK_ARG(cols % 4 == 0 && ld % 4 == 0 && (reinterpret_cast<uintptr_t>(src) % 16) == 0 &&
                    (reinterpret_cast<uintptr_t>(dst) % 8) == 0,
                "dxa_split3: cols and ld must be multiples of 4 and the buffers 16-byte aligned");
  hipLaunchKernelGGL(split3_k, dim3(dxa_grid1d(rows * (cols / 4), 256)), dim3(256), 0, (hipStream_t)stream, src, ld,
                     (bf16_t*)dst, rows, cols, side);
  DXA_CHECK_LAUNCH();
  return DXA_OK;
}

#if defined(DXA_PP3_STAMPS)
extern "C" int dxa_gemm_debug_pp3_stamps(unsigned long long* out) {
  DXA_CHECK_HIP(hipDeviceSynchronize());
  DXA_CHECK_HIP(hipMemcpyFromSymbol(out, HIP_SYMBOL(g_pp3_stamps), sizeof(unsigned long long) * 4));
  return DXA_OK;
}
#endif
```

### dexbotic_amd/csrc/gemm_common.h

```cpp
#pragma once
#include "common.h"

namespace dxa_gemm_detail {
typedef float f32x16_t __attribute__((ext_vector_type(16)));
struct GemmP {
  int64_t M, N, K;
  const char* A; int64_t lda;
  const char* B; int64_t ldb;
  char* C; int64_t ldc;
  const char* bias;
  const char* R; int64_t ldr;
  char* aux;
  const char* G; int64_t ldg;
  float alpha;
  int act, accumulate;
  int nb1, nb2;
  int64_t sA[3], sB[3], sC[3], sR[3], sG[3];
  int tm, tn;
  int vecA, vecB, vecC, vecR, vecG, vecBias;
  int full, tail_r, split_s;
  int group_m;
  char* mirror;
  float* sumsq;
  float* ws;
  int* flags;
  const char* A2; const char* B2; int64_t K2;
  int fuse; int64_t ldaux;
};
}

namespace {
using dxa_gemm_detail::GemmP;
using dxa_gemm_detail::f32x16_t;
typedef uint32_t u32x4n_t __attribute__((ext_vector_type(4)));
typedef uint32_t u32x4_t __attribute__((ext_vector_type(4)));
typedef __attribute__((address_space(3))) void lds_void_t;
constexpr int BM = 128, BN = 128;
constexpr int ROWB = 128;
constexpr int TILE_BYTES = BM * ROWB;

template <typename T> __device__ __forceinline__ void load4(float (&o)[4], const T* p, bool vec, int n_ok);
template <> __device__ __forceinline__ void load4<float>(float (&o)[4], const float* p, bool vec, int n_ok) {
  if (vec && n_ok == 4) {
    const float4 v = *reinterpret_cast<const float4*>(p);
    o[0] = v.x; o[1] = v.y; o[2] = v.z; o[3] = v.w;
  } else {
#pragma unroll
    for (int i = 0; i < 4; ++i) o[i] = i < n_ok ? p[i] : 0.f;
  }
}
template <> __device__ __forceinline__ void load4<bf16_t>(float (&o)[4], const bf16_t* p, bool vec, int n_ok) {
  if (vec && n_ok == 4) {
    const uint2 v = *reinterpret_cast<const uint2*>(p);
    o[0] = __uint_as_float(v.x << 16); o[1] = __uint_as_float(v.x & 0xffff0000u);
    o[2] = __uint_as_float(v.y << 16); o[3] = __uint_as_float(v.y & 0xffff0000u);
  } else {
#pragma unroll
    for (int i = 0; i < 4; ++i) o[i] = i < n_ok ? bf2f(p[i]) : 0.f;
  }
}
template <typename T> __device__ __forceinline__ void store4(T* p, const float (&v)[4], bool vec, int n_ok);
template <> __device__ __forceinline__ void store4<float>(float* p, const float (&v)[4], bool vec, int n_ok) {
  if (vec && n_ok == 4) {
    *reinterpret_cast<float4*>(p) = make_float4(v[0], v[1], v[2], v[3]);
  } else {
#pragma unroll
    for (int i = 0; i < 4; ++i) if (i < n_ok) p[i] = v[i];
  }
}
template <> __device__ __forceinline__ void store4<bf16_t>(bf16_t* p, const float (&v)[4], bool vec, int n_ok) {
  if (vec && n_ok == 4) {
    uint2 o;
    o.x = pack_bf16x2(v[0], v[1]);
    o.y = pack_bf16x2(v[2], v[3]);
    *reinterpret_cast<uint2*>(p) = o;
  } else {
#pragma unroll
    for (int i = 0; i < 4; ++i) if (i < n_ok) p[i] = f2bf(v[i]);
  }
}

template <typename TI, typename TO>
__device__ __forceinline__ void epilogue4(const GemmP& p, TO* C, TO* AUX, const TI* R, const TI* G,
                                          const float (&bv)[4], int64_t m, int64_t n, int n_ok, const float (&a)[4]) {
  float v[4];
#pragma unroll
  for (int r = 0; r < 4; ++r) v[r] = a[r] * p.alpha + bv[r];
  if (AUX) store4<TO>(AUX + m * p.ldc + n, v, p.vecC, n_ok);
  if (G) {
    float g[4];
    load4<TI>(g, G + m * p.ldg + n, p.vecG, n_ok);
#pragma unroll
    for (int r = 0; r < 4; ++r) v[r] *= act_grad(p.act, g[r]);
  } else if (p.act != DXA_ACT_NONE) {
#pragma unroll
    for (int r = 0; r < 4; ++r) v[r] = act_fwd(p.act, v[r]);
  }
  if (R) {
    float rr[4];
    load4<TI>(rr, R + m * p.ldr + n, p.vecR, n_ok);
#pragma unroll
    for (int r = 0; r < 4; ++r) v[r] += rr[r];
  }
  TO* cp = C + m * p.ldc + n;
  if (p.accumulate) {
    float c0[4];
    load4<TO>(c0, cp, p.vecC, n_ok);
#pragma unroll
    for (int r = 0; r < 4; ++r) v[r] += c0[r];
  }
  store4<TO>(cp, v, p.vecC, n_ok);
}

constexpr int NUM_CU_D = 256;

template <int AI>
__device__ __forceinline__ bool tile_split_exchange(const GemmP& p, f32x16_t (&acc)[AI][2], int tid, int split_j, int split_s,
                                                    int tail_i) {
#if defined(__HIP_DEVICE_COMPILE__)
  if (split_s > 1) {
    constexpr int SC1 = 16;
    constexpr uint32_t SLOT = 256 * 256 * 4;
    const __amdgpu_buffer_rsrc_t rW = __builtin_amdgcn_make_buffer_rsrc(p.ws, 0, (int)(NUM_CU_D * SLOT), 0x00020000);
    const uint32_t slot0 = (uint32_t)tail_i * (uint32_t)(split_s - 1) * SLOT + (uint32_t)tid * 16u;
    if (split_j < split_s - 1) {
      const uint32_t dst = slot0 + (uint32_t)split_j * SLOT;
#pragma unroll
      for (int i = 0; i < AI; ++i)
#pragma unroll
        for (int j = 0; j < 2; ++j)
#pragma unroll
          for (int q = 0; q < 4; ++q) {
            const f32x4_t v = {acc[i][j][4 * q], acc[i][j][4 * q + 1], acc[i][j][4 * q + 2], acc[i][j][4 * q + 3]};
            __builtin_amdgcn_raw_buffer_store_b128(__builtin_bit_cast(u32x4_t, v), rW, dst + ((i * 2 + j) * 4 + q) * 8192, 0, SC1);
          }
      asm volatile("s_waitcnt vmcnt(0)" ::: "memory");
      __syncthreads();
      if (tid == 0) __hip_atomic_fetch_add(p.flags + tail_i, 1, __ATOMIC_RELAXED, __HIP_MEMORY_SCOPE_AGENT);
      return false;
    }
    if (tid == 0) {
      while (__hip_atomic_load(p.flags + tail_i, __ATOMIC_RELAXED, __HIP_MEMORY_SCOPE_AGENT) < split_s - 1)
        __builtin_amdgcn_s_sleep(4);
      __hip_atomic_store(p.flags + tail_i, 0, __ATOMIC_RELAXED, __HIP_MEMORY_SCOPE_AGENT);
    }
    __syncthreads();
    for (int sj = 0; sj < split_s - 1; ++sj) {
      const uint32_t src = slot0 + (uint32_t)sj * SLOT;
#pragma unroll
      for (int i = 0; i < AI; ++i) {
#pragma unroll
        for (int j = 0; j < 2; ++j)
#pragma unroll
          for (int q = 0; q < 4; ++q) {
            const f32x4_t v = __builtin_bit_cast(f32x4_t, __builtin_amdgcn_raw_buffer_load_b128(rW, src + ((i * 2 + j) * 4 + q) * 8192, 0, SC1));
#pragma unroll
            for (int c = 0; c < 4; ++c) acc[i][j][4 * q + c] += v[c];
          }
        if (AI == 4 && i == 1) __builtin_amdgcn_sched_barrier(0);
      }
    }
  }

#endif
  return true;
}

template <typename TO, int AI, typename TE, bool SMALL = false>
__device__ __forceinline__ void tile_finish(const GemmP& p, f32x16_t (&acc)[AI][2], char* smem, int tid, int lane, int wave,
                                            int wm, int wn, int l32, int lh, int64_t m0, int64_t n0, int split_j,
                                            int split_s, int tail_i) {
#if defined(__HIP_DEVICE_COMPILE__)
  constexpr int BMR = AI * 64;
  if (!tile_split_exchange<AI>(p, acc, tid, split_j, split_s, tail_i)) return;

  TO* C = reinterpret_cast<TO*>(p.C);
  TO* AUX = p.aux ? reinterpret_cast<TO*>(p.aux) : nullptr;
  const TE* R = reinterpret_cast<const TE*>(p.R);
  const TE* G = reinterpret_cast<const TE*>(p.G);
  const TE* bias = reinterpret_cast<const TE*>(p.bias);
  const int cr = lane >> 4, cc = (lane & 15) * 4;
  const int64_t n = n0 + wn * 64 + cc;
  const int n_ok = (int)max((int64_t)0, min((int64_t)4, p.N - n));
  float bv[4] = {0.f, 0.f, 0.f, 0.f};
  if (bias && n_ok > 0) load4<TE>(bv, bias + n, p.vecBias, n_ok);
  if constexpr (!SMALL) {
    constexpr int ROWP = 64 * 4 + 16;
    char* slab = smem + wave * (64 * ROWP);
#pragma unroll
    for (int pass = 0; pass < 2; ++pass) {
#pragma unroll
      for (int ii = 0; ii < 2; ++ii)
#pragma unroll
        for (int j = 0; j < 2; ++j)
#pragma unroll
          for (int q = 0; q < 4; ++q) {
            const int i = 2 * pass + ii;
            if (i >= AI) continue;
            float4 v = make_float4(acc[i][j][4 * q], acc[i][j][4 * q + 1], acc[i][j][4 * q + 2], acc[i][j][4 * q + 3]);
            *reinterpret_cast<float4*>(slab + (ii * 32 + l32) * ROWP + (j * 32 + 8 * q + 4 * lh) * 4) = v;
          }
      __builtin_amdgcn_fence(__ATOMIC_RELEASE, "wavefront");
      __builtin_amdgcn_wave_barrier();
#pragma unroll 4
      for (int it = 0; it < (AI == 3 && pass == 1 ? 8 : 16); ++it) {
        const int row = cr + 4 * it;
        const int64_t m = m0 + wm * (BMR / 2) + pass * 64 + row;
        const float4 v = *reinterpret_cast<const float4*>(slab + row * ROWP + cc * 4);
        if (m < p.M && n_ok > 0) {
          const float a4[4] = {v.x, v.y, v.z, v.w};
          epilogue4<TE, TO>(p, C, AUX, R, G, bv, m, n, n_ok, a4);
        }
      }
      __builtin_amdgcn_fence(__ATOMIC_RELEASE, "wavefront");
      __builtin_amdgcn_wave_barrier();
    }
  } else {
    char* slab = smem + 131072 + wave * 4096;
    const int r16 = l32 & 15;
#pragma unroll
    for (int i = 0; i < AI; ++i)
#pragma unroll
      for (int hh = 0; hh < 2; ++hh) {
        if ((l32 >> 4) == hh) {
#pragma unroll
          for (int j = 0; j < 2; ++j)
#pragma unroll
            for (int q = 0; q < 4; ++q) {
              float4 v = make_float4(acc[i][j][4 * q], acc[i][j][4 * q + 1], acc[i][j][4 * q + 2], acc[i][j][4 * q + 3]);
              *reinterpret_cast<float4*>(slab + r16 * 256 + (((j * 8 + 2 * q + lh) ^ r16) << 4)) = v;
            }
        }
        __builtin_amdgcn_fence(__ATOMIC_RELEASE, "wavefront");
        __builtin_amdgcn_wave_barrier();
#pragma unroll
        for (int it = 0; it < 4; ++it) {
          const int row = cr + 4 * it;
          const int64_t m = m0 + wm * (BMR / 2) + i * 32 + hh * 16 + row;
          const float4 v = *reinterpret_cast<const float4*>(slab + row * 256 + (((lane & 15) ^ row) << 4));
          if (m < p.M && n_ok > 0) {
            const float a4[4] = {v.x, v.y, v.z, v.w};
            epilogue4<TE, TO>(p, C, AUX, R, G, bv, m, n, n_ok, a4);
          }
        }
        __builtin_amdgcn_fence(__ATOMIC_RELEASE, "wavefront");
        __builtin_amdgcn_wave_barrier();
        __builtin_amdgcn_sched_barrier(0);
      }
  }
#endif
}

__device__ __forceinline__ void sk_tile_origin(const GemmP& p, int t, int& m0, int& n0) {
  const int width = p.group_m * p.tn;
  const int group = t / width;
  const int first_pm = group * p.group_m;
  const int gsz = min(p.tm - first_pm, p.group_m);
  const int rem = t - group * width;
  const int pn = rem / gsz;
  m0 = (first_pm + rem - pn * gsz) * 256;
  n0 = pn * 256;
}
template <typename T> struct SkIO;
template <> struct SkIO<float> {
  template <int CPL>
  static __device__ __forceinline__ void ld(float (&o)[CPL], __amdgpu_buffer_rsrc_t r, uint32_t off) {
    static_assert(CPL == 4, "fp32 operands come 4 columns per lane");
    const f32x4_t v = __builtin_bit_cast(f32x4_t, __builtin_amdgcn_raw_buffer_load_b128(r, off, 0, 0));
#pragma unroll
    for (int e = 0; e < 4; ++e) o[e] = v[e];
  }
  template <int CPL>
  static __device__ __forceinline__ void st(const float (&v)[CPL], __amdgpu_buffer_rsrc_t r, uint32_t off) {
    static_assert(CPL == 4, "fp32 outputs go 4 columns per lane");
    const f32x4_t o = {v[0], v[1], v[2], v[3]};
    __builtin_amdgcn_raw_buffer_store_b128(__builtin_bit_cast(u32x4_t, o), r, off, 0, 0);
  }
};
template <> struct SkIO<bf16_t> {
  template <int CPL>
  static __device__ __forceinline__ void ld(float (&o)[CPL], __amdgpu_buffer_rsrc_t r, uint32_t off) {
    if constexpr (CPL == 8) {
      const u32x4_t v = __builtin_amdgcn_raw_buffer_load_b128(r, off, 0, 0);
#pragma unroll
      for (int e = 0; e < 4; ++e) { o[2 * e] = __uint_as_float(v[e] << 16); o[2 * e + 1] = __uint_as_float(v[e] & 0xffff0000u); }
    } else {
      typedef uint32_t u32x2_t __attribute__((ext_vector_type(2)));
      const u32x2_t v = __builtin_amdgcn_raw_buffer_load_b64(r, off, 0, 0);
#pragma unroll
      for (int e = 0; e < 2; ++e) { o[2 * e] = __uint_as_float(v[e] << 16); o[2 * e + 1] = __uint_as_float(v[e] & 0xffff0000u); }
    }
  }
  template <int CPL>
  static __device__ __forceinline__ void st(const float (&v)[CPL], __amdgpu_buffer_rsrc_t r, uint32_t off) {
    static_assert(CPL == 8, "bf16 outputs go 8 columns per lane");
    u32x4_t o;
#pragma unroll
    for (int e = 0; e < 4; ++e) o[e] = pack_bf16x2(v[2 * e], v[2 * e + 1]);
    __builtin_amdgcn_raw_buffer_store_b128(o, r, off, 0, 0);
  }
};

template <typename TO, typename TE, int AI = 4>
__device__ __forceinline__ float sk_epilogue_rows(const GemmP& p, f32x16_t (&acc)[AI][2], char* slab, int lane, int wm, int wn,
                                                  int m0, int n0) {
  float ssq = 0.f;
#if defined(__HIP_DEVICE_COMPILE__)
  constexpr int CPL = 16 / (int)sizeof(TO);
  constexpr int LPR = 64 / CPL;
  constexpr int RPI = 64 / LPR;
  const int l32 = lane & 31, lh = lane >> 5, r16 = l32 & 15;
  const int lr = lane / LPR, lc = (lane % LPR) * CPL;
  const int n = n0 + wn * 64 + lc;
  const int rowb = m0 + wm * (32 * AI) + lr;
  const bool col_ok = n < (int)p.N;
  const uint32_t Mi = (uint32_t)p.M;
  const uint32_t esO = sizeof(TO), esE = sizeof(TE);
  const __amdgpu_buffer_rsrc_t rC = __builtin_amdgcn_make_buffer_rsrc(p.C, 0, (int)(((p.M - 1) * p.ldc + p.N) * esO), 0x00020000);
  const __amdgpu_buffer_rsrc_t rR = __builtin_amdgcn_make_buffer_rsrc(const_cast<char*>(p.R ? p.R : p.A), 0, p.R ? (int)(((p.M - 1) * p.ldr + p.N) * esE) : 0, 0x00020000);
  const uint32_t ldcB = (uint32_t)p.ldc * esO, ldrB = (uint32_t)p.ldr * esE;
  const uint32_t offC0 = (uint32_t)rowb * ldcB + (uint32_t)n * esO;
  const uint32_t offR0 = (uint32_t)rowb * ldrB + (uint32_t)n * esE;
  float bv[CPL];
#pragma unroll
  for (int e = 0; e < CPL; ++e) bv[e] = 0.f;
  if (p.bias && col_ok) {
    const __amdgpu_buffer_rsrc_t rBias = __builtin_amdgcn_make_buffer_rsrc(const_cast<char*>(p.bias), 0, (int)(p.N * esE), 0x00020000);
    SkIO<TE>::template ld<CPL>(bv, rBias, (uint32_t)n * esE);
  }
  const bool has_R = p.R != nullptr, accum = p.accumulate != 0, has_mirror = p.mirror != nullptr;
  const __amdgpu_buffer_rsrc_t rM = __builtin_amdgcn_make_buffer_rsrc(p.mirror ? p.mirror : (char*)p.C, 0,
                                                                      p.mirror ? (int)(((p.M - 1) * p.ldc + p.N) * 2) : 0, 0x00020000);
  const float alpha = p.alpha;
  const bool want_ssq = p.sumsq != nullptr;
#pragma unroll
  for (int i = 0; i < AI; ++i)
#pragma unroll
    for (int hh = 0; hh < 2; ++hh) {
      if ((l32 >> 4) == hh) {
#pragma unroll
        for (int j = 0; j < 2; ++j)
#pragma unroll
          for (int q = 0; q < 4; ++q) {
            float4 v = make_float4(acc[i][j][4 * q], acc[i][j][4 * q + 1], acc[i][j][4 * q + 2], acc[i][j][4 * q + 3]);
            *reinterpret_cast<float4*>(slab + r16 * 256 + (((j * 8 + 2 * q + lh) ^ r16) << 4)) = v;
          }
      }
      __builtin_amdgcn_fence(__ATOMIC_RELEASE, "wavefront");
      __builtin_amdgcn_wave_barrier();
#pragma unroll
      for (int it = 0; it < 16 / RPI; ++it) {
        const int row = lr + RPI * it;
        const uint32_t rr = (uint32_t)(32 * i + 16 * hh + RPI * it);
        const bool ok = col_ok && (uint32_t)rowb + rr < Mi;
        float v[CPL];
#pragma unroll
        for (int u = 0; u < CPL / 4; ++u) {
          const float4 t = *reinterpret_cast<const float4*>(slab + row * 256 + (((lc / 4 + u) ^ row) << 4));
          v[4 * u] = t.x; v[4 * u + 1] = t.y; v[4 * u + 2] = t.z; v[4 * u + 3] = t.w;
        }
        const uint32_t oc = ok ? offC0 + rr * ldcB : 0x80000000u;
#pragma unroll
        for (int e = 0; e < CPL; ++e) v[e] = v[e] * alpha + bv[e];
        if (has_R) {
          float r[CPL];
          SkIO<TE>::template ld<CPL>(r, rR, ok ? offR0 + rr * ldrB : 0x80000000u);
#pragma unroll
          for (int e = 0; e < CPL; ++e) v[e] += r[e];
        }
        if (accum) {
          float c0[CPL];
          SkIO<TO>::template ld<CPL>(c0, rC, oc);
#pragma unroll
          for (int e = 0; e < CPL; ++e) v[e] += c0[e];
        }
        SkIO<TO>::template st<CPL>(v, rC, oc);
        if constexpr (sizeof(TO) == 2) {
          if (want_ssq && ok) {
#pragma unroll
            for (int e = 0; e < CPL; ++e) { const float t = rnd<bf16_t>(v[e]); ssq += t * t; }
          }
        }
        if constexpr (sizeof(TO) == 4) {
          if (ok) {
#pragma unroll
            for (int e = 0; e < CPL; ++e) ssq += v[e] * v[e];
          }
          if (has_mirror) {
            typedef uint32_t u32x2_t_ __attribute__((ext_vector_type(2)));
            const u32x2_t_ o2 = {pack_bf16x2(v[0], v[1]), pack_bf16x2(v[2], v[3])};
            __builtin_amdgcn_raw_buffer_store_b64(o2, rM, ok ? (offC0 + rr * ldcB) >> 1 : 0x80000000u, 0, 0);
          }
        }
      }
      __builtin_amdgcn_fence(__ATOMIC_RELEASE, "wavefront");
      __builtin_amdgcn_wave_barrier();
      __builtin_amdgcn_sched_barrier(0);
    }
#endif
  return ssq;
}
template <int AI = 4>
__device__ __forceinline__ void sk_epilogue_swiglu(const GemmP& p, f32x16_t (&acc)[AI][2], char* slab, int lane, int wm, int wn,
                                                   int m0, int n0) {
#if defined(__HIP_DEVICE_COMPILE__)
  const int l32 = lane & 31, lh = lane >> 5, r16 = l32 & 15;
  const int lr = lane >> 3, lq = lane & 7;
  const int F = (int)(p.N >> 1);
  const int nout = (n0 >> 1) + wn * 32 + lq * 4;
  const int rowb = m0 + wm * (32 * AI) + lr;
  const bool col_ok = nout < F;
  const uint32_t Mi = (uint32_t)p.M;
  const __amdgpu_buffer_rsrc_t rC = __builtin_amdgcn_make_buffer_rsrc(p.C, 0, (int)(((p.M - 1) * p.ldc + F) * 2), 0x00020000);
  const __amdgpu_buffer_rsrc_t rX = __builtin_amdgcn_make_buffer_rsrc(p.aux ? p.aux : p.C, 0,
                                                                      p.aux ? (int)(((p.M - 1) * p.ldaux + p.N) * 2) : 0, 0x00020000);
  const uint32_t ldcB = (uint32_t)p.ldc * 2u, ldxB = (uint32_t)p.ldaux * 2u;
  const uint32_t offC0 = (uint32_t)rowb * ldcB + (uint32_t)nout * 2u;
  const uint32_t offG0 = (uint32_t)rowb * ldxB + (uint32_t)nout * 2u, offU0 = offG0 + (uint32_t)F * 2u;
  const bool has_aux = p.aux != nullptr;
  const float alpha = p.alpha;
  typedef uint32_t u32x2_t_ __attribute__((ext_vector_type(2)));
#pragma unroll
  for (int i = 0; i < AI; ++i)
#pragma unroll
    for (int hh = 0; hh < 2; ++hh) {
      if ((l32 >> 4) == hh) {
#pragma unroll
        for (int j = 0; j < 2; ++j)
#pragma unroll
          for (int q = 0; q < 4; ++q) {
            float4 v = make_float4(acc[i][j][4 * q], acc[i][j][4 * q + 1], acc[i][j][4 * q + 2], acc[i][j][4 * q + 3]);
            *reinterpret_cast<float4*>(slab + r16 * 256 + (((j * 8 + 2 * q + lh) ^ r16) << 4)) = v;
          }
      }
      __builtin_amdgcn_fence(__ATOMIC_RELEASE, "wavefront");
      __builtin_amdgcn_wave_barrier();
#pragma unroll
      for (int it = 0; it < 2; ++it) {
        const int row = lr + 8 * it;
        const uint32_t rr = (uint32_t)(32 * i + 16 * hh + 8 * it);
        const bool ok = col_ok && (uint32_t)rowb + rr < Mi;
        const float4 g4 = *reinterpret_cast<const float4*>(slab + row * 256 + ((lq ^ row) << 4));
        const float4 u4 = *reinterpret_cast<const float4*>(slab + row * 256 + (((8 + lq) ^ row) << 4));
        const float g[4] = {rnd<bf16_t>(g4.x * alpha + 0.f), rnd<bf16_t>(g4.y * alpha + 0.f), rnd<bf16_t>(g4.z * alpha + 0.f), rnd<bf16_t>(g4.w * alpha + 0.f)};
        const float u[4] = {rnd<bf16_t>(u4.x * alpha + 0.f), rnd<bf16_t>(u4.y * alpha + 0.f), rnd<bf16_t>(u4.z * alpha + 0.f), rnd<bf16_t>(u4.w * alpha + 0.f)};
        float o[4];
#pragma unroll
        for (int e = 0; e < 4; ++e) {
          o[e] = rnd<bf16_t>(g[e] * fast_sigmoidf(g[e])) * u[e];
        }
        const u32x2_t_ ov = {pack_bf16x2(o[0], o[1]), pack_bf16x2(o[2], o[3])};
        __builtin_amdgcn_raw_buffer_store_b64(ov, rC, ok ? offC0 + rr * ldcB : 0x80000000u, 0, 0);
        if (has_aux) {
          const u32x2_t_ gv = {pack_bf16x2(g[0], g[1]), pack_bf16x2(g[2], g[3])};
          const u32x2_t_ uv = {pack_bf16x2(u[0], u[1]), pack_bf16x2(u[2], u[3])};
          __builtin_amdgcn_raw_buffer_store_b64(gv, rX, ok ? offG0 + rr * ldxB : 0x80000000u, 0, 0);
          __builtin_amdgcn_raw_buffer_store_b64(uv, rX, ok ? offU0 + rr * ldxB : 0x80000000u, 0, 0);
        }
      }
      __builtin_amdgcn_fence(__ATOMIC_RELEASE, "wavefront");
      __builtin_amdgcn_wave_barrier();
      __builtin_amdgcn_sched_barrier(0);
    }
#endif
}
template <typename TO, typename TE, int AI = 4>
__device__ __forceinline__ void sk_epilogue(const GemmP& p, f32x16_t (&acc)[AI][2], char* slab, int lane, int wm, int wn,
                                            int m0, int n0, float* red, int tile) {
#if defined(__HIP_DEVICE_COMPILE__)
  float ssq = sk_epilogue_rows<TO, TE, AI>(p, acc, slab, lane, wm, wn, m0, n0);
  {
    if (p.sumsq != nullptr) {
#pragma unroll
      for (int o = 32; o > 0; o >>= 1) ssq += __shfl_xor(ssq, o, 64);
      if (lane == 0) red[wm * 4 + wn] = ssq;
      __syncthreads();
      if (threadIdx.x == 0) {
        float t = 0.f;
#pragma unroll
        for (int w8 = 0; w8 < 8; ++w8) t += red[w8];
        p.sumsq[tile] = t;
      }
    }
  }
#endif
}
}
```

Baseline: 70.43 episodes/s.

## Switch ping-pong GEMM main loop from 32x32x16 to 16x16x32 MFMA

```diff
diff --git a/dexbotic_amd/csrc/gemm.hip b/dexbotic_amd/csrc/gemm.hip
--- a/dexbotic_amd/csrc/gemm.hip
+++ b/dexbotic_amd/csrc/gemm.hip
@@ -881,7 +881,7 @@
 #pragma unroll
       for (int j = 0; j < 2; ++j) {
         const int krow = (wave * 2 + j) * 4 + (lane >> 4);
-        const int sig = (lane & 15) ^ ((krow & 3) << 2);
+        const int sig = (lane & 15) ^ ((krow & 3) << 2) ^ (((krow >> 3) & 1) << 1);
         if constexpr (A_KS) {
           const int ga = m0i + (sig >> 3) * 128 + 64 * h + 8 * (sig & 7);
           voA[h][j] = ga < (int)p.M ? (uint32_t)krow * lda2 + (uint32_t)ga * 2u : 0x80000000u;
@@ -943,23 +943,20 @@
 #define PP_DMA_A(h, buf, tile) do { PP_DMA_A1(h, 0, buf, tile); PP_DMA_A1(h, 1, buf, tile); } while (0)
 #define PP_DMA_B(h, buf, tile) do { PP_DMA_B1(h, 0, buf, tile); PP_DMA_B1(h, 1, buf, tile); } while (0)
 
-  f32x16_t acc[4][2];
-#pragma unroll
-  for (int i = 0; i < 4; ++i)
-#pragma unroll
-    for (int j = 0; j < 2; ++j)
-#pragma unroll
-      for (int r = 0; r < 16; ++r) acc[i][j][r] = 0.f;
+  f32x4_t acc[8][4];
+#pragma unroll
+  for (int i = 0; i < 8; ++i)
+#pragma unroll
+    for (int j = 0; j < 4; ++j) acc[i][j] = (f32x4_t){0.f, 0.f, 0.f, 0.f};
 
   const uint32_t lds0 = (uint32_t)(uintptr_t)(__attribute__((address_space(3))) char*)smem;
-  const int sw = (l32 >> 1) & 7;
-  const int i16 = lane & 15, tq = (i16 >> 2) & 3, tk = 8 * lh + (i16 >> 2);
-  const uint32_t ks_lane = (uint32_t)(tk * 256 + ((lane >> 4) & 1) * 32 + (i16 & 3) * 8);
+  const int i16 = lane & 15, g = lane >> 4, sw = (i16 >> 1) & 7, tq = (i16 >> 2) & 3;
+  const uint32_t ks_lane = (uint32_t)((8 * g + (i16 >> 2)) * 256 + (g & 1) * 32 + (i16 & 3) * 8);
   const uint32_t ya = A_KS ? lds0 + ks_lane + (uint32_t)(((wm * 2) ^ tq) << 6)
-                           : (lds0 + (wm * 128 + l32) * 128) | (uint32_t)((lh ^ sw) << 4);
+                           : (lds0 + (wm * 128 + i16) * 128) | (uint32_t)((g ^ sw) << 4);
   const uint32_t yb = B_KS ? lds0 + REG + ks_lane + (uint32_t)((wn ^ tq) << 6)
-                           : (lds0 + REG + (wn * 64 + l32) * 128) | (uint32_t)((lh ^ sw) << 4);
-  u32x4_t af[2][4], bq[2][4];
+                           : (lds0 + REG + (wn * 64 + i16) * 128) | (uint32_t)((g ^ sw) << 4);
+  u32x4_t af[4][2], bq[2][2][2];
   typedef uint32_t u32x2_t __attribute__((ext_vector_type(2)));
 #define PP_READ(dst, addr, imm) asm volatile("ds_read_b128 %0, %1 offset:%2" : "=v"(dst) : "v"(addr), "n"(imm) : "memory")
 #define PP_READ_TR(dst, addr, imm) asm volatile("ds_read_b64_tr_b16 %0, %1 offset:%2" : "=v"(dst) : "v"(addr), "n"(imm) : "memory")
@@ -969,78 +966,30 @@
     PP_READ_TR(lo_, addr, imm); PP_READ_TR(hi_, addr, (imm) + 1024);                     \
     dst = (u32x4_t){lo_[0], lo_[1], hi_[0], hi_[1]};                                     \
   } while (0)
-#define PP_RD_A(cur, h)                                                                                     \
+#define PP_RDF_A(cur, h, b, ks)                                                                             \
   do {                                                                                                      \
-    if constexpr (A_KS) {                                                                                   \
-      const uint32_t a0_ = ya ^ (uint32_t)((cur) * BUF + (h) * 16384), a1_ = a0_ ^ 64u;                     \
-      PP_FRAG_TR(af[0][0], a0_, 0); PP_FRAG_TR(af[1][0], a1_, 0);                                           \
-      PP_FRAG_TR(af[0][1], a0_, 4096); PP_FRAG_TR(af[1][1], a1_, 4096);                                     \
-      PP_FRAG_TR(af[0][2], a0_, 8192); PP_FRAG_TR(af[1][2], a1_, 8192);                                     \
-      PP_FRAG_TR(af[0][3], a0_, 12288); PP_FRAG_TR(af[1][3], a1_, 12288);                                   \
-    } else {                                                                                                \
-      const uint32_t a0_ = ya ^ (uint32_t)((cur) * BUF), a1_ = ya ^ (uint32_t)((cur) * BUF + 32),           \
-                     a2_ = ya ^ (uint32_t)((cur) * BUF + 64), a3_ = ya ^ (uint32_t)((cur) * BUF + 96);      \
-      PP_READ(af[0][0], a0_, (2 * (h)) * 4096); PP_READ(af[1][0], a0_, (2 * (h) + 1) * 4096);              \
-      PP_READ(af[0][1], a1_, (2 * (h)) * 4096); PP_READ(af[1][1], a1_, (2 * (h) + 1) * 4096);              \
-      PP_READ(af[0][2], a2_, (2 * (h)) * 4096); PP_READ(af[1][2], a2_, (2 * (h) + 1) * 4096);              \
-      PP_READ(af[0][3], a3_, (2 * (h)) * 4096); PP_READ(af[1][3], a3_, (2 * (h) + 1) * 4096);              \
-    }                                                                                                       \
+    if constexpr (A_KS) PP_FRAG_TR(af[b][ks], ya ^ (uint32_t)((cur) * BUF + 32 * (b)), (h) * 16384 + (ks) * 8192); \
+    else PP_READ(af[b][ks], ya ^ (uint32_t)((cur) * BUF + 64 * (ks)), (4 * (h) + (b)) * 2048);            \
   } while (0)
-#define PP_RD_B(cur, j)                                                                                     \
+#define PP_RDF_B(cur, j, b, ks)                                                                             \
   do {                                                                                                      \
-    if constexpr (B_KS) {                                                                                   \
-      const uint32_t b0_ = yb ^ (uint32_t)((cur) * BUF + (j) * 16384);                                      \
-      PP_FRAG_TR(bq[j][0], b0_, 0); PP_FRAG_TR(bq[j][1], b0_, 4096);                                        \
-      PP_FRAG_TR(bq[j][2], b0_, 8192); PP_FRAG_TR(bq[j][3], b0_, 12288);                                    \
-    } else {                                                                                                \
-      const uint32_t b0_ = yb ^ (uint32_t)((cur) * BUF), b1_ = yb ^ (uint32_t)((cur) * BUF + 32),           \
-                     b2_ = yb ^ (uint32_t)((cur) * BUF + 64), b3_ = yb ^ (uint32_t)((cur) * BUF + 96);      \
-      PP_READ(bq[j][0], b0_, (j) * 4096); PP_READ(bq[j][1], b1_, (j) * 4096);                               \
-      PP_READ(bq[j][2], b2_, (j) * 4096); PP_READ(bq[j][3], b3_, (j) * 4096);                               \
-    }                                                                                                       \
+    if constexpr (B_KS) PP_FRAG_TR(bq[j][b][ks], yb ^ (uint32_t)((cur) * BUF + 32 * (b)), (j) * 16384 + (ks) * 8192); \
+    else PP_READ(bq[j][b][ks], yb ^ (uint32_t)((cur) * BUF + 64 * (ks)), (2 * (j) + (b)) * 2048);         \
   } while (0)
-#define PP_MFMA(ii, ks, i, j) acc[i][j] = __builtin_amdgcn_mfma_f32_32x32x16_bf16(__builtin_bit_cast(bf16x8_t, bq[j][ks]), __builtin_bit_cast(bf16x8_t, af[ii][ks]), acc[i][j], 0, 0, 0)
+#define PP_MFMA(h, j, b, jb, ks)                                                                                            \
+  acc[4 * (h) + (b)][2 * (j) + (jb)] = __builtin_amdgcn_mfma_f32_16x16x32_bf16(                                           \
+      __builtin_bit_cast(bf16x8_t, bq[j][jb][ks]), __builtin_bit_cast(bf16x8_t, af[b][ks]), acc[4 * (h) + (b)][2 * (j) + (jb)], 0, 0, 0)
 #define PP_SB() __builtin_amdgcn_sched_barrier(0)
 #define PP_BAR() do { PP_SB(); __builtin_amdgcn_s_barrier(); PP_SB(); } while (0)
-#define PP_COMPUTE(h, j)                                                                          \
-  do {                                                                                            \
-    asm volatile("s_waitcnt lgkmcnt(0)" ::: "memory");                                            \
-    PP_SB();                                                                                      \
-    PP_MFMA(0, 0, 2 * (h), j); PP_MFMA(1, 0, 2 * (h) + 1, j);                                     \
-    PP_MFMA(0, 1, 2 * (h), j); PP_MFMA(1, 1, 2 * (h) + 1, j);                                     \
-    PP_MFMA(0, 2, 2 * (h), j); PP_MFMA(1, 2, 2 * (h) + 1, j);                                     \
-    PP_MFMA(0, 3, 2 * (h), j); PP_MFMA(1, 3, 2 * (h) + 1, j);                                     \
-    PP_SB();                                                                                      \
-  } while (0)
-#define PP_RDK_A(cur, h, ks)                                                                                \
-  do {                                                                                                      \
-    if constexpr (A_KS) {                                                                                   \
-      const uint32_t a0_ = ya ^ (uint32_t)((cur) * BUF + (h) * 16384), a1_ = a0_ ^ 64u;                     \
-      PP_FRAG_TR(af[0][ks], a0_, 4096 * (ks)); PP_FRAG_TR(af[1][ks], a1_, 4096 * (ks));                     \
-    } else {                                                                                                \
-      const uint32_t a_ = ya ^ (uint32_t)((cur) * BUF + 32 * (ks));                                         \
-      PP_READ(af[0][ks], a_, (2 * (h)) * 4096); PP_READ(af[1][ks], a_, (2 * (h) + 1) * 4096);              \
-    }                                                                                                       \
-  } while (0)
-#define PP_RDK_B(cur, j, ks)                                                                                \
-  do {                                                                                                      \
-    if constexpr (B_KS) {                                                                                   \
-      const uint32_t b0_ = yb ^ (uint32_t)((cur) * BUF + (j) * 16384);                                      \
-      PP_FRAG_TR(bq[j][ks], b0_, 4096 * (ks));                                                              \
-    } else {                                                                                                \
-      const uint32_t b_ = yb ^ (uint32_t)((cur) * BUF + 32 * (ks));                                         \
-      PP_READ(bq[j][ks], b_, (j) * 4096);                                                                   \
-    }                                                                                                       \
-  } while (0)
+#define PP_MFMA2(h, j, b, ks, R) do { PP_MFMA(h, j, b, 0, ks); PP_MFMA(h, j, b, 1, ks); PP_SB(); R(ks, b); PP_SB(); } while (0)
 #define PP_COMPUTE_R(h, j, R)                                                                     \
   do {                                                                                            \
     asm volatile("s_waitcnt lgkmcnt(0)" ::: "memory");                                            \
     PP_SB();                                                                                      \
-    PP_MFMA(0, 0, 2 * (h), j); PP_MFMA(1, 0, 2 * (h) + 1, j); PP_SB(); R(0); PP_SB();             \
-    PP_MFMA(0, 1, 2 * (h), j); PP_MFMA(1, 1, 2 * (h) + 1, j); PP_SB(); R(1); PP_SB();             \
-    PP_MFMA(0, 2, 2 * (h), j); PP_MFMA(1, 2, 2 * (h) + 1, j); PP_SB(); R(2); PP_SB();             \
-    PP_MFMA(0, 3, 2 * (h), j); PP_MFMA(1, 3, 2 * (h) + 1, j); PP_SB(); R(3); PP_SB();             \
+    PP_MFMA2(h, j, 0, 0, R); PP_MFMA2(h, j, 1, 0, R); PP_MFMA2(h, j, 2, 0, R); PP_MFMA2(h, j, 3, 0, R); \
+    PP_MFMA2(h, j, 0, 1, R); PP_MFMA2(h, j, 1, 1, R); PP_MFMA2(h, j, 2, 1, R); PP_MFMA2(h, j, 3, 1, R); \
   } while (0)
+#define PP_R_NONE(ks, b) do { } while (0)
 #define PP_VMCNT(n) asm volatile("s_waitcnt vmcnt(" #n ")" ::: "memory")
 #if defined(DXA_PP_STAMPS)
   uint64_t ts_[8];
@@ -1059,9 +1008,16 @@
 #define PP_STAMP(i) do { } while (0)
 #define PP_STAMPS_FOLD() do { } while (0)
 #endif
-#define PP_R_B1(ks) PP_RDK_B(cur_, 1, ks)
-#define PP_R_A1(ks) PP_RDK_A(cur_, 1, ks)
-#define PP_R_NEXT(ks) do { if (more1) { PP_RDK_A(cur_ ^ 1, 0, ks); PP_RDK_B(cur_ ^ 1, 0, ks); } } while (0)
+#define PP_R_B1(ks, b) do { if constexpr (((b) & 1) != 0) PP_RDF_B(cur_, 1, (b) >> 1, ks); } while (0)
+#define PP_R_A1(ks, b) PP_RDF_A(cur_, 1, b, ks)
+#define PP_R_NEXT(ks, b)                                                                                    \
+  do {                                                                                                      \
+    if (more1) {                                                                                            \
+      PP_RDF_A(cur_ ^ 1, 0, b, ks);                                                                         \
+      if constexpr ((ks) == 1 && (b) < 2) PP_RDF_B(cur_ ^ 1, 0, (b) & 1, 0);                                \
+      if constexpr ((ks) == 1 && (b) == 3) { PP_RDF_B(cur_ ^ 1, 0, 0, 1); PP_RDF_B(cur_ ^ 1, 0, 1, 1); }    \
+    }                                                                                                       \
+  } while (0)
 #define PP_TILE(cur, t)                                                                                     \
   do {                                                                                                      \
     constexpr int cur_ = (cur);                                                                             \
@@ -1074,7 +1030,7 @@
     PP_BAR(); PP_STAMP(2); PP_COMPUTE_R(0, 1, PP_R_A1); PP_BAR(); PP_STAMP(3);                              \
                                                                                                \
     if (more2) { PP_DMA_B(0, cur_, (t) + 2); PP_SB(); PP_VMCNT(8); } else if (more1) { PP_VMCNT(4); }       \
-    PP_BAR(); PP_STAMP(4); PP_COMPUTE(1, 1); PP_BAR(); PP_STAMP(5);                                         \
+    PP_BAR(); PP_STAMP(4); PP_COMPUTE_R(1, 1, PP_R_NONE); PP_BAR(); PP_STAMP(5);                                         \
                                                                                                \
     if (more2) { PP_DMA_B(1, cur_, (t) + 2); PP_SB(); PP_VMCNT(8); } else if (more1) { PP_VMCNT(2); }       \
     PP_BAR(); PP_STAMP(6); PP_COMPUTE_R(1, 0, PP_R_NEXT); PP_BAR(); PP_STAMP(7);                            \
@@ -1086,7 +1042,9 @@
   PP_SB();
   if (nk > 1) { PP_VMCNT(8); } else { PP_VMCNT(2); }
   PP_BAR();
-  PP_RD_A(0, 0); PP_RD_B(0, 0);
+  PP_RDF_A(0, 0, 0, 0); PP_RDF_A(0, 0, 1, 0); PP_RDF_A(0, 0, 2, 0); PP_RDF_A(0, 0, 3, 0);
+  PP_RDF_A(0, 0, 0, 1); PP_RDF_A(0, 0, 1, 1); PP_RDF_A(0, 0, 2, 1); PP_RDF_A(0, 0, 3, 1);
+  PP_RDF_B(0, 0, 0, 0); PP_RDF_B(0, 0, 1, 0); PP_RDF_B(0, 0, 0, 1); PP_RDF_B(0, 0, 1, 1);
   PP_SB();
   if (wm == 1) PP_BAR();
   for (int t = 0; t < nk; t += 2) {
@@ -1105,30 +1063,29 @@
 #undef PP_READ
 #undef PP_READ_TR
 #undef PP_FRAG_TR
-#undef PP_RD_A
-#undef PP_RD_B
+#undef PP_RDF_A
+#undef PP_RDF_B
 #undef PP_MFMA
+#undef PP_MFMA2
 #undef PP_SB
 #undef PP_BAR
-#undef PP_COMPUTE
+#undef PP_R_NONE
 #undef PP_VMCNT
 #undef PP_TILE
 #undef PP_DMA_A1
 #undef PP_DMA_B1
 #undef PP_STAMP
 #undef PP_STAMPS_FOLD
-#undef PP_RDK_A
-#undef PP_RDK_B
 #undef PP_COMPUTE_R
 #undef PP_R_B1
 #undef PP_R_A1
 #undef PP_R_NEXT
 
   if constexpr (LEAN) {
-    if (!tile_split_exchange<4>(p, acc, tid, split_j, split_s, tail_i)) return;
+    if (!tile_split_exchange<4, 16>(p, acc, tid, split_j, split_s, tail_i)) return;
     __builtin_amdgcn_sched_barrier(0);
-    if constexpr (FUSE == 1) sk_epilogue_swiglu<4>(p, acc, smem + wave * 4096, lane, wm, wn, m0i, n0i);
-    else sk_epilogue<TO, TE>(p, acc, smem + wave * 4096, lane, wm, wn, m0i, n0i, reinterpret_cast<float*>(smem + 8 * 4096), bid);
+    if constexpr (FUSE == 1) sk_epilogue_swiglu<4, 16>(p, acc, smem + wave * 4096, lane, wm, wn, m0i, n0i);
+    else sk_epilogue<TO, TE, 4, 16>(p, acc, smem + wave * 4096, lane, wm, wn, m0i, n0i, reinterpret_cast<float*>(smem + 8 * 4096), bid);
 #if defined(DXA_PP_STAMPS)
     __syncthreads();
     if (m0i == 0 && n0i == 0 && lane == 0) {
@@ -1138,7 +1095,7 @@
     }
 #endif
   } else {
-    tile_finish<TO, 4, TE>(p, acc, smem, tid, lane, wave, wm, wn, l32, lh, m0, n0, split_j, split_s, tail_i);
+    tile_finish<TO, 4, TE, false, 16>(p, acc, smem, tid, lane, wave, wm, wn, l32, lh, m0, n0, split_j, split_s, tail_i);
   }
 #endif
 }
diff --git a/dexbotic_amd/csrc/gemm_common.h b/dexbotic_amd/csrc/gemm_common.h
--- a/dexbotic_amd/csrc/gemm_common.h
+++ b/dexbotic_amd/csrc/gemm_common.h
@@ -114,10 +114,40 @@
 
 constexpr int NUM_CU_D = 256;
 
-template <int AI>
-__device__ __forceinline__ bool tile_split_exchange(const GemmP& p, f32x16_t (&acc)[AI][2], int tid, int split_j, int split_s,
+template <int AI, int MF> struct AccL;
+template <int AI> struct AccL<AI, 32> { typedef f32x16_t T[AI][2]; };
+template <int AI> struct AccL<AI, 16> {
+  typedef f32x4_t T[2 * AI][4];
+  static __device__ __forceinline__ f32x4_t unit(const T& a, int u) { return a[u >> 2][u & 3]; }
+  static __device__ __forceinline__ void add(T& a, int u, const f32x4_t& v) { a[u >> 2][u & 3] += v; }
+  static __device__ __forceinline__ void stage16(const T& a, int s, char* slab, int lane) {
+    const int r16 = lane & 15, g = lane >> 4;
+#pragma unroll
+    for (int j = 0; j < 4; ++j) {
+      const f32x4_t x = a[s][j];
+      *reinterpret_cast<float4*>(slab + r16 * 256 + (((j * 4 + g) ^ r16) << 4)) = make_float4(x[0], x[1], x[2], x[3]);
+    }
+  }
+  template <int RP>
+  static __device__ __forceinline__ void stage64(const T& a, int s, char* slab, int lane) {
+    const int r16 = lane & 15, g = lane >> 4;
+#pragma unroll
+    for (int ii = 0; ii < 4; ++ii)
+#pragma unroll
+      for (int j = 0; j < 4; ++j) {
+        const int i = 4 * s + ii;
+        if (i >= 2 * AI) continue;
+        const f32x4_t x = a[i][j];
+        *reinterpret_cast<float4*>(slab + (ii * 16 + r16) * RP + (j * 16 + 4 * g) * 4) = make_float4(x[0], x[1], x[2], x[3]);
+      }
+  }
+};
+
+template <int AI, int MF = 32>
+__device__ __forceinline__ bool tile_split_exchange(const GemmP& p, typename AccL<AI, MF>::T& acc, int tid, int split_j, int split_s,
                                                     int tail_i) {
 #if defined(__HIP_DEVICE_COMPILE__)
+  typedef AccL<AI, MF> L;
   if (split_s > 1) {
     constexpr int SC1 = 16;
     constexpr uint32_t SLOT = 256 * 256 * 4;
@@ -125,15 +155,21 @@
     const uint32_t slot0 = (uint32_t)tail_i * (uint32_t)(split_s - 1) * SLOT + (uint32_t)tid * 16u;
     if (split_j < split_s - 1) {
       const uint32_t dst = slot0 + (uint32_t)split_j * SLOT;
-#pragma unroll
-      for (int i = 0; i < AI; ++i)
-#pragma unroll
-        for (int j = 0; j < 2; ++j)
-#pragma unroll
-          for (int q = 0; q < 4; ++q) {
-            const f32x4_t v = {acc[i][j][4 * q], acc[i][j][4 * q + 1], acc[i][j][4 * q + 2], acc[i][j][4 * q + 3]};
-            __builtin_amdgcn_raw_buffer_store_b128(__builtin_bit_cast(u32x4_t, v), rW, dst + ((i * 2 + j) * 4 + q) * 8192, 0, SC1);
-          }
+      if constexpr (MF == 32) {
+#pragma unroll
+        for (int i = 0; i < AI; ++i)
+#pragma unroll
+          for (int j = 0; j < 2; ++j)
+#pragma unroll
+            for (int q = 0; q < 4; ++q) {
+              const f32x4_t v = {acc[i][j][4 * q], acc[i][j][4 * q + 1], acc[i][j][4 * q + 2], acc[i][j][4 * q + 3]};
+              __builtin_amdgcn_raw_buffer_store_b128(__builtin_bit_cast(u32x4_t, v), rW, dst + ((i * 2 + j) * 4 + q) * 8192, 0, SC1);
+            }
+      } else {
+#pragma unroll
+        for (int u = 0; u < 8 * AI; ++u)
+          __builtin_amdgcn_raw_buffer_store_b128(__builtin_bit_cast(u32x4_t, L::unit(acc, u)), rW, dst + u * 8192, 0, SC1);
+      }
       asm volatile("s_waitcnt vmcnt(0)" ::: "memory");
       __syncthreads();
       if (tid == 0) __hip_atomic_fetch_add(p.flags + tail_i, 1, __ATOMIC_RELAXED, __HIP_MEMORY_SCOPE_AGENT);
@@ -147,17 +183,25 @@
     __syncthreads();
     for (int sj = 0; sj < split_s - 1; ++sj) {
       const uint32_t src = slot0 + (uint32_t)sj * SLOT;
-#pragma unroll
-      for (int i = 0; i < AI; ++i) {
-#pragma unroll
-        for (int j = 0; j < 2; ++j)
-#pragma unroll
-          for (int q = 0; q < 4; ++q) {
-            const f32x4_t v = __builtin_bit_cast(f32x4_t, __builtin_amdgcn_raw_buffer_load_b128(rW, src + ((i * 2 + j) * 4 + q) * 8192, 0, SC1));
-#pragma unroll
-            for (int c = 0; c < 4; ++c) acc[i][j][4 * q + c] += v[c];
-          }
-        if (AI == 4 && i == 1) __builtin_amdgcn_sched_barrier(0);
+      if constexpr (MF == 32) {
+#pragma unroll
+        for (int i = 0; i < AI; ++i) {
+#pragma unroll
+          for (int j = 0; j < 2; ++j)
+#pragma unroll
+            for (int q = 0; q < 4; ++q) {
+              const f32x4_t v = __builtin_bit_cast(f32x4_t, __builtin_amdgcn_raw_buffer_load_b128(rW, src + ((i * 2 + j) * 4 + q) * 8192, 0, SC1));
+#pragma unroll
+              for (int c = 0; c < 4; ++c) acc[i][j][4 * q + c] += v[c];
+            }
+          if (AI == 4 && i == 1) __builtin_amdgcn_sched_barrier(0);
+        }
+      } else {
+#pragma unroll
+        for (int u = 0; u < 8 * AI; ++u) {
+          L::add(acc, u, __builtin_bit_cast(f32x4_t, __builtin_amdgcn_raw_buffer_load_b128(rW, src + u * 8192, 0, SC1)));
+          if (AI == 4 && u == 15) __builtin_amdgcn_sched_barrier(0);
+        }
       }
     }
   }
@@ -166,13 +210,14 @@
   return true;
 }
 
-template <typename TO, int AI, typename TE, bool SMALL = false>
-__device__ __forceinline__ void tile_finish(const GemmP& p, f32x16_t (&acc)[AI][2], char* smem, int tid, int lane, int wave,
+template <typename TO, int AI, typename TE, bool SMALL = false, int MF = 32>
+__device__ __forceinline__ void tile_finish(const GemmP& p, typename AccL<AI, MF>::T& acc, char* smem, int tid, int lane, int wave,
                                             int wm, int wn, int l32, int lh, int64_t m0, int64_t n0, int split_j,
                                             int split_s, int tail_i) {
 #if defined(__HIP_DEVICE_COMPILE__)
+  typedef AccL<AI, MF> L;
   constexpr int BMR = AI * 64;
-  if (!tile_split_exchange<AI>(p, acc, tid, split_j, split_s, tail_i)) return;
+  if (!tile_split_exchange<AI, MF>(p, acc, tid, split_j, split_s, tail_i)) return;
 
   TO* C = reinterpret_cast<TO*>(p.C);
   TO* AUX = p.aux ? reinterpret_cast<TO*>(p.aux) : nullptr;
@@ -189,17 +234,21 @@
     char* slab = smem + wave * (64 * ROWP);
 #pragma unroll
     for (int pass = 0; pass < 2; ++pass) {
-#pragma unroll
-      for (int ii = 0; ii < 2; ++ii)
-#pragma unroll
-        for (int j = 0; j < 2; ++j)
-#pragma unroll
-          for (int q = 0; q < 4; ++q) {
-            const int i = 2 * pass + ii;
-            if (i >= AI) continue;
-            float4 v = make_float4(acc[i][j][4 * q], acc[i][j][4 * q + 1], acc[i][j][4 * q + 2], acc[i][j][4 * q + 3]);
-            *reinterpret_cast<float4*>(slab + (ii * 32 + l32) * ROWP + (j * 32 + 8 * q + 4 * lh) * 4) = v;
-          }
+      if constexpr (MF == 32) {
+#pragma unroll
+        for (int ii = 0; ii < 2; ++ii)
+#pragma unroll
+          for (int j = 0; j < 2; ++j)
+#pragma unroll
+            for (int q = 0; q < 4; ++q) {
+              const int i = 2 * pass + ii;
+              if (i >= AI) continue;
+              float4 v = make_float4(acc[i][j][4 * q], acc[i][j][4 * q + 1], acc[i][j][4 * q + 2], acc[i][j][4 * q + 3]);
+              *reinterpret_cast<float4*>(slab + (ii * 32 + l32) * ROWP + (j * 32 + 8 * q + 4 * lh) * 4) = v;
+            }
+      } else {
+        L::template stage64<ROWP>(acc, pass, slab, lane);
+      }
       __builtin_amdgcn_fence(__ATOMIC_RELEASE, "wavefront");
       __builtin_amdgcn_wave_barrier();
 #pragma unroll 4
@@ -217,19 +266,23 @@
     }
   } else {
     char* slab = smem + 131072 + wave * 4096;
-    const int r16 = l32 & 15;
+    [[maybe_unused]] const int r16 = l32 & 15;
 #pragma unroll
     for (int i = 0; i < AI; ++i)
 #pragma unroll
       for (int hh = 0; hh < 2; ++hh) {
-        if ((l32 >> 4) == hh) {
-#pragma unroll
-          for (int j = 0; j < 2; ++j)
-#pragma unroll
-            for (int q = 0; q < 4; ++q) {
-              float4 v = make_float4(acc[i][j][4 * q], acc[i][j][4 * q + 1], acc[i][j][4 * q + 2], acc[i][j][4 * q + 3]);
-              *reinterpret_cast<float4*>(slab + r16 * 256 + (((j * 8 + 2 * q + lh) ^ r16) << 4)) = v;
-            }
+        if constexpr (MF == 32) {
+          if ((l32 >> 4) == hh) {
+#pragma unroll
+            for (int j = 0; j < 2; ++j)
+#pragma unroll
+              for (int q = 0; q < 4; ++q) {
+                float4 v = make_float4(acc[i][j][4 * q], acc[i][j][4 * q + 1], acc[i][j][4 * q + 2], acc[i][j][4 * q + 3]);
+                *reinterpret_cast<float4*>(slab + r16 * 256 + (((j * 8 + 2 * q + lh) ^ r16) << 4)) = v;
+              }
+          }
+        } else {
+          L::stage16(acc, 2 * i + hh, slab, lane);
         }
         __builtin_amdgcn_fence(__ATOMIC_RELEASE, "wavefront");
         __builtin_amdgcn_wave_barrier();
@@ -301,15 +354,15 @@
   }
 };
 
-template <typename TO, typename TE, int AI = 4>
-__device__ __forceinline__ float sk_epilogue_rows(const GemmP& p, f32x16_t (&acc)[AI][2], char* slab, int lane, int wm, int wn,
+template <typename TO, typename TE, int AI = 4, int MF = 32>
+__device__ __forceinline__ float sk_epilogue_rows(const GemmP& p, typename AccL<AI, MF>::T& acc, char* slab, int lane, int wm, int wn,
                                                   int m0, int n0) {
   float ssq = 0.f;
 #if defined(__HIP_DEVICE_COMPILE__)
   constexpr int CPL = 16 / (int)sizeof(TO);
   constexpr int LPR = 64 / CPL;
   constexpr int RPI = 64 / LPR;
-  const int l32 = lane & 31, lh = lane >> 5, r16 = l32 & 15;
+  [[maybe_unused]] const int l32 = lane & 31, lh = lane >> 5, r16 = l32 & 15;
   const int lr = lane / LPR, lc = (lane % LPR) * CPL;
   const int n = n0 + wn * 64 + lc;
   const int rowb = m0 + wm * (32 * AI) + lr;
@@ -337,14 +390,18 @@
   for (int i = 0; i < AI; ++i)
 #pragma unroll
     for (int hh = 0; hh < 2; ++hh) {
-      if ((l32 >> 4) == hh) {
-#pragma unroll
-        for (int j = 0; j < 2; ++j)
-#pragma unroll
-          for (int q = 0; q < 4; ++q) {
-            float4 v = make_float4(acc[i][j][4 * q], acc[i][j][4 * q + 1], acc[i][j][4 * q + 2], acc[i][j][4 * q + 3]);
-            *reinterpret_cast<float4*>(slab + r16 * 256 + (((j * 8 + 2 * q + lh) ^ r16) << 4)) = v;
-          }
+      if constexpr (MF == 32) {
+        if ((l32 >> 4) == hh) {
+#pragma unroll
+          for (int j = 0; j < 2; ++j)
+#pragma unroll
+            for (int q = 0; q < 4; ++q) {
+              float4 v = make_float4(acc[i][j][4 * q], acc[i][j][4 * q + 1], acc[i][j][4 * q + 2], acc[i][j][4 * q + 3]);
+              *reinterpret_cast<float4*>(slab + r16 * 256 + (((j * 8 + 2 * q + lh) ^ r16) << 4)) = v;
+            }
+        }
+      } else {
+        AccL<AI, MF>::stage16(acc, 2 * i + hh, slab, lane);
       }
       __builtin_amdgcn_fence(__ATOMIC_RELEASE, "wavefront");
       __builtin_amdgcn_wave_barrier();
@@ -400,11 +457,11 @@
 #endif
   return ssq;
 }
-template <int AI = 4>
-__device__ __forceinline__ void sk_epilogue_swiglu(const GemmP& p, f32x16_t (&acc)[AI][2], char* slab, int lane, int wm, int wn,
+template <int AI = 4, int MF = 32>
+__device__ __forceinline__ void sk_epilogue_swiglu(const GemmP& p, typename AccL<AI, MF>::T& acc, char* slab, int lane, int wm, int wn,
                                                    int m0, int n0) {
 #if defined(__HIP_DEVICE_COMPILE__)
-  const int l32 = lane & 31, lh = lane >> 5, r16 = l32 & 15;
+  [[maybe_unused]] const int l32 = lane & 31, lh = lane >> 5, r16 = l32 & 15;
   const int lr = lane >> 3, lq = lane & 7;
   const int F = (int)(p.N >> 1);
   const int nout = (n0 >> 1) + wn * 32 + lq * 4;
@@ -424,14 +481,18 @@
   for (int i = 0; i < AI; ++i)
 #pragma unroll
     for (int hh = 0; hh < 2; ++hh) {
-      if ((l32 >> 4) == hh) {
-#pragma unroll
-        for (int j = 0; j < 2; ++j)
-#pragma unroll
-          for (int q = 0; q < 4; ++q) {
-            float4 v = make_float4(acc[i][j][4 * q], acc[i][j][4 * q + 1], acc[i][j][4 * q + 2], acc[i][j][4 * q + 3]);
-            *reinterpret_cast<float4*>(slab + r16 * 256 + (((j * 8 + 2 * q + lh) ^ r16) << 4)) = v;
-          }
+      if constexpr (MF == 32) {
+        if ((l32 >> 4) == hh) {
+#pragma unroll
+          for (int j = 0; j < 2; ++j)
+#pragma unroll
+            for (int q = 0; q < 4; ++q) {
+              float4 v = make_float4(acc[i][j][4 * q], acc[i][j][4 * q + 1], acc[i][j][4 * q + 2], acc[i][j][4 * q + 3]);
+              *reinterpret_cast<float4*>(slab + r16 * 256 + (((j * 8 + 2 * q + lh) ^ r16) << 4)) = v;
+            }
+        }
+      } else {
+        AccL<AI, MF>::stage16(acc, 2 * i + hh, slab, lane);
       }
       __builtin_amdgcn_fence(__ATOMIC_RELEASE, "wavefront");
       __builtin_amdgcn_wave_barrier();
@@ -464,11 +525,11 @@
     }
 #endif
 }
-template <typename TO, typename TE, int AI = 4>
-__device__ __forceinline__ void sk_epilogue(const GemmP& p, f32x16_t (&acc)[AI][2], char* slab, int lane, int wm, int wn,
+template <typename TO, typename TE, int AI = 4, int MF = 32>
+__device__ __forceinline__ void sk_epilogue(const GemmP& p, typename AccL<AI, MF>::T& acc, char* slab, int lane, int wm, int wn,
                                             int m0, int n0, float* red, int tile) {
 #if defined(__HIP_DEVICE_COMPILE__)
-  float ssq = sk_epilogue_rows<TO, TE, AI>(p, acc, slab, lane, wm, wn, m0, n0);
+  float ssq = sk_epilogue_rows<TO, TE, AI, MF>(p, acc, slab, lane, wm, wn, m0, n0);
   {
     if (p.sumsq != nullptr) {
 #pragma unroll
```

Result: faster. 71.83 episodes/s (median of 6 runs) (+2.0%).
